# dek226/CSE375-FinalProj-Huffman-Decoding

Measured on AMD Instinct MI355X. Metric: decoded GB/s, higher is better.
Workload: dtype u8

## Files before the change

cse375-finalproj-huffman-decoding_amd/csrc/gh_decode.hip:

```cpp
#include <hip/hip_runtime.h>
#include <hip/hip_ext.h>

#include <algorithm>
#include <cmath>
#include <cstdio>
#include <cstring>
#include <map>
#include <memory>
#include <mutex>
#include <string>
#include <thread>
#include <type_traits>
#include <vector>

#include "gh_device.hpp"
#include "gh_gather_range.hpp"
#include "gh_hip.hpp"
#include "gh_internal.hpp"
#include "gh_lut.hpp"

namespace gh {

constexpr uint32_t EPOCH_MAX = (1u << 24) - 1;

#include "gh_tile.hip"
#include "gh_wsplit.hip"
#include "gh_index.hip"
#include "gh_gather.hip"
#include "gh_gather_plan.hip"
#include "gh_mtile.hip"

}

using namespace gh;

static uint32_t tile_u_for(uint32_t minlen) { return minlen >= 4 ? (uint32_t)TILE_U : (uint32_t)TILE_U3; }
#ifndef GH_TILE_OW7
#define GH_TILE_OW7 1
#endif
struct Kern {
  const void* fn;
  const char* name;
};
template <class... A>
static std::string kern_name(const char* fmt, A... a) {
  char b[96];
  snprintf(b, sizeof(b), fmt, a...);
  return b;
}
template <int TB, int U, int G, int OW, int MINL>
static Kern tile_kern() {
  static const std::string n = kern_name("tile<%d,%d,%d,%d,%d>", TB, U, G, OW, MINL);
  return {(const void*)gh_tile_kernel<TB, U, G, OW, MINL>, n.c_str()};
}
template <int TB, int GL, int NS, bool FB, int NP = 1>
static Kern mtile_kern() {
  static const std::string n = kern_name("mtile<%d,%d,%d,fb=%d,np=%d>", TB, GL, NS, (int)FB, NP);
  return {(const void*)gh_mtile_kernel<TB, GL, NS, FB, NP>, n.c_str()};
}
template <int U, int TB, int GL, bool FB>
static Kern ws_count_kern() {
  static const std::string n = kern_name("ws_count<%d,%d,%d,fb=%d>", U, TB, GL, (int)FB);
  return {(const void*)gh_ws_count_kernel<U, TB, GL, FB>, n.c_str()};
}
template <int U, int TB, int GL, int NS, bool FB>
static Kern ws_write_kern() {
  static const std::string n = kern_name("ws_write<%d,%d,%d,%d,fb=%d>", U, TB, GL, NS, (int)FB);
  return {(const void*)gh_ws_write_kernel<U, TB, GL, NS, FB>, n.c_str()};
}

static Kern tile_kernel_for(uint32_t minlen, uint32_t g) {
  if (minlen >= 5 && GH_TILE_OW7)
    return g >= 4 ? tile_kern<TILE_TB, TILE_U, 4, 7, 5>()
         : g == 3 ? tile_kern<TILE_TB, TILE_U, 3, 7, 5>()
                  : tile_kern<TILE_TB, TILE_U, 2, 7, 5>();
  if (minlen >= 4)
    return g >= 4 ? tile_kern<TILE_TB, TILE_U, 4, 8, 4>()
         : g == 3 ? tile_kern<TILE_TB, TILE_U, 3, 8, 4>()
                  : tile_kern<TILE_TB, TILE_U, 2, 8, 4>();
  return g >= 4 ? tile_kern<TILE_TB, TILE_U3, 4, 11, 3>()
       : g == 3 ? tile_kern<TILE_TB, TILE_U3, 3, 11, 3>()
                : tile_kern<TILE_TB, TILE_U3, 2, 11, 3>();
}

template <int GL, bool FB>
static Kern mtile_ns(int ns) {
  return ns <= 4 ? mtile_kern<MT_TB, GL, 4, FB>()
       : ns <= 6 ? mtile_kern<MT_TB, GL, 6, FB>()
       : ns <= 8 ? mtile_kern<MT_TB, GL, 8, FB>()
                 : mtile_kern<MT_TB, GL, 5, FB, 2>();
}
static Kern mtile_kernel_for(int gl, int ns, bool fb = false) {
  if (fb) return mtile_ns<2, true>(ns);
  return gl >= 4 ? mtile_ns<4, false>(ns) : gl == 3 ? mtile_ns<3, false>(ns) : mtile_ns<2, false>(ns);
}

struct WsKernels {
  Kern count;
  Kern write;
};
template <int GL, bool FB = false>
static Kern ws_write_ns(int ns) {
  return ns <= 2 ? ws_write_kern<WS_U, WS_TB, GL, 2, FB>()
         : ns <= 3 ? ws_write_kern<WS_U, WS_TB, GL, 3, FB>()
         : ns <= 4 ? ws_write_kern<WS_U, WS_TB, GL, 4, FB>()
         : ns <= 6 ? ws_write_kern<WS_U, WS_TB, GL, 6, FB>()
                   : ws_write_kern<WS_U, WS_TB, GL, 8, FB>();
}
template <class F>
static auto kernel_by_width(uint32_t bits, bool fb, F kern) {
  using std::integral_constant;
  if (fb) return kern(integral_constant<int, 2>{}, std::true_type{});
  const int gl = lookups_per_shift(bits);
  return gl >= 4 ? kern(integral_constant<int, 4>{}, std::false_type{})
       : gl == 3 ? kern(integral_constant<int, 3>{}, std::false_type{})
                 : kern(integral_constant<int, 2>{}, std::false_type{});
}
static WsKernels ws_kernels(uint32_t Kc, uint32_t K, int ns, bool fb) {
  return {kernel_by_width(Kc, fb, [](auto gl, auto f) { return ws_count_kern<WS_UC, WS_TBC, decltype(gl)::value, decltype(f)::value>(); }),
          kernel_by_width(K, fb, [ns](auto gl, auto f) { return ws_write_ns<decltype(gl)::value, decltype(f)::value>(ns); })};
}

static std::string all_kernel_shapes() {
  std::vector<std::string> v;
  auto add = [&](const char* n) {
    if (std::find(v.begin(), v.end(), n) == v.end()) v.push_back(n);
  };
  for (uint32_t ml = 3; ml <= 12; ++ml)
    for (uint32_t g = 2; g <= 4; ++g) add(tile_kernel_for(ml, g).name);
  for (int fb = 0; fb <= 1; ++fb)
    for (int gl = 2; gl <= 4; ++gl)
      for (int ns = 4; ns <= 10; ++ns) add(mtile_kernel_for(gl, ns, fb != 0).name);
  for (int pass = 0; pass < 2; ++pass)
    for (int fb = 0; fb <= 1; ++fb)
      for (uint32_t kc = 2; kc <= 14; ++kc)
        for (uint32_t k = 2; k <= 12; ++k)
          for (int ns = 2; ns <= 8; ++ns) {
            const WsKernels w = ws_kernels(kc, k, ns, fb != 0);
            add(pass ? w.write.name : w.count.name);
          }
  std::string s;
  for (const std::string& n : v) s += n + "\n";
  return s;
}

static_assert(TILE_U <= 4 && TILE_U3 <= 4, "payload padding (16 words) covers at most 4 segments per lane");


struct Shard {
  uint64_t nseg = 0, seg_begin = 0, seg_end = 0, n_total = 0, g_total = 0;
  uint32_t gap_nib0 = 0, first_start = 0;
  uint32_t last_end = 0;
  DevBuf payload;
  DevBuf gaps;
  DevBuf out;
  uint64_t out_cap = 0;
};

enum class Mode { NONE, TILE, MTILE, WSPLIT };

struct TilePlan {
  uint32_t ntiles = 0;
  uint32_t kbits = 0;
  uint32_t kbits_c = 0;
  uint32_t lut_lgr = 0;
  uint32_t clut_lgr = 0;
  uint32_t lut_bytes = 0;
  uint32_t stage_bytes = 0;
  uint32_t idle_block = 0xFFFFFFFFu;
  uint32_t epoch = 0;
  uint64_t gran_words = 0;
  DevBuf lut;
  DevBuf gran;
  DevBuf stamps;
};

struct WsPlan {
  Kern count{};
  uint32_t grid_c = 0;
  size_t lds_count = 0;
  uint32_t k = 0, kc = 0;
  uint32_t lgc = 0;
  uint32_t lut_bytes = 0;
  uint32_t stage_bytes = 0;
  uint32_t nblocks = 0, nranges = 0;
  DevBuf lut_c;
  DevBuf lut_w;
  DevBuf fb;
  DevBuf seg_cnt, junk, rng_tot, rng_off;
};

struct Plan {
  Mode mode = Mode::NONE;
  Kern kern{};
  uint32_t grid = 0, block = 0;
  size_t lds = 0;
  std::string shape;
  TilePlan tile;
  WsPlan ws;
  bool tiled() const { return mode == Mode::TILE || mode == Mode::MTILE; }
};

struct GatherTables {
  bool ready = false;
  uint32_t kc = 0, ks = 0;
  uint32_t last_end = 0;
  uint32_t wgs = 0;
  size_t lds = 0;
  const void* kern = nullptr;
  DevBuf lut_c;
  DevBuf lut_s;
  DevBuf fb;
};
struct Gather {
  GatherTables tab;
  DevBuf d_pieces, d_out;
  std::vector<gh_gather_piece> pieces;
  EventPair ev;
};
struct DevGather {
  bool has_index = false;
  uint32_t log2_stride = 0;
  uint64_t nblocks = 0;
  DevBuf offsets, rank;
  DevBuf loc, slot, dst0, pieces;
  Event ev_a, ev_b, ev_c;
  bool enqueued = false;
  hipStream_t last_stream = nullptr;
};

struct Timing {
  std::vector<EventPair> pending, pool;
  double acc_ms = 0;
  uint32_t nlaunch = 0;
};

struct gh_ctx {
  int device = 0;
  int num_cu = 0;
  Stream stream;
  Event done;
  bool done_rec = false;
  hipEvent_t done_ev = nullptr;
  bool loaded = false;
  Canon canon;
  DevBuf misc;
  Shard shard;
  Plan plan;
  Gather gather;
  DevGather dgather;
  Timing timing;
  ~gh_ctx();
  unsigned int* misc_at(int i) const { return misc.get<unsigned int>() + i; }
};

static void free_shard(gh_ctx* c) {
  (void)hipSetDevice(c->device);
  c->shard = Shard{};
  c->plan = Plan{};
  c->gather.tab = GatherTables{};
  c->dgather.has_index = false;
  c->dgather.offsets.reset();
  c->dgather.rank.reset();
  c->dgather.enqueued = false;
  c->loaded = false;
}

static int allow_lds(const void* fn, size_t lds) {
  if (lds > 64 * 1024) GH_HIP(hipFuncSetAttribute(fn, hipFuncAttributeMaxDynamicSharedMemorySize, (int)lds));
  return GH_OK;
}


static uint32_t tile_grid_cap(uint32_t grid) {
  if (const char* e = getenv("GH_TILE_GRID"))
    if (grid > 2) return (uint32_t)std::clamp<long>(atol(e), 2, (long)grid);
  return grid;
}

static int tile_grid_and_granules(Plan& p, uint64_t resident) {
  p.grid = (uint32_t)std::min<uint64_t>({(uint64_t)p.tile.ntiles + 1, resident, (uint64_t)LEAD_A * p.block});
  p.grid = tile_grid_cap(p.grid);
  if (p.grid < 2) return GH_OK;
  p.tile.gran_words = 2ull * p.tile.ntiles + 2;
  return p.tile.gran.alloc(8ull * p.tile.gran_words, true);
}

static int tile_setup(gh_ctx* c, uint32_t K, double avg_seg_bytes) {
  const Canon& cn = c->canon;
  Plan p;
  TilePlan& t = p.tile;
  const uint32_t maxsyms = (128 + cn.minlen - 1) / cn.minlen;
  t.kbits = K;
  const uint32_t tile_u = tile_u_for(cn.minlen);
  t.ntiles = (uint32_t)ceil_div(c->shard.nseg, (uint64_t)tile_u * TILE_TB);
  double scapf = 1.12;
  if (const char* e = getenv("GH_TILE_SCAPF")) scapf = std::clamp(atof(e), 0.5, 4.0);
  uint64_t per_seg = std::min<uint64_t>(
      maxsyms, cn.minlen >= 4 ? (uint64_t)TILE_SCAP : (uint64_t)std::ceil(std::max(avg_seg_bytes, 1.0) * scapf + 1));
  if (const char* e = getenv("GH_TILE_SCAP")) per_seg = std::min<uint64_t>(maxsyms, (uint64_t)std::max(1, atoi(e)));
  const uint64_t margin = 4ull * (cn.minlen >= 4 ? 8 : 11) + 4;
  const uint64_t seg_wave = 64ull * tile_u;
  per_seg = std::min<uint64_t>(per_seg, ((uint64_t)TILE_NS * 64 * 16 - 2 * STAGE_PAD - margin) / seg_wave);
  t.stage_bytes = (uint32_t)((STAGE_PAD + seg_wave * per_seg + margin + 15) & ~15ull);
  const std::vector<uint32_t> lt = grouped_lut(cn, K);
  p.kern = tile_kernel_for(cn.minlen, std::min<uint32_t>(4, 32 / cn.maxlen));
  p.block = TILE_TB;
  if (int rc = allow_lds(p.kern.fn, 160 * 1024)) return rc;
  const char* envr = getenv("GH_LGR");
  const int lg = envr ? std::clamp(atoi(envr), 0, 14 - (int)K) : std::min(5, 14 - (int)K);
  int best = 0, best_lg = 0;
  for (int l2 = lg; l2 >= 0; --l2) {
    int pc = 0;
    GH_HIP(hipOccupancyMaxActiveBlocksPerMultiprocessor(&pc, p.kern.fn, TILE_TB, tile_lds_bytes(4ull << (K + l2), t.stage_bytes)));
    if (pc > best) {
      best = pc;
      best_lg = l2;
    }
    if (envr) break;
  }
  best = std::min(best, 2);
  if (best < 1) return GH_OK;
  t.lut_lgr = (uint32_t)best_lg;
  t.lut_bytes = (uint32_t)(4ull << (K + best_lg));
  p.lds = tile_lds_bytes(t.lut_bytes, t.stage_bytes);
  if (int rc = tile_grid_and_granules(p, (uint64_t)best * c->num_cu)) return rc;
  if (p.grid < 2) return GH_OK;
  if (const char* e = getenv("GH_TILE_IDLE"))
    if (atoi(e) && p.grid == (uint32_t)best * c->num_cu && best == 2) t.idle_block = p.grid / 2;
  if (int rc = t.lut.upload(lt.data(), 4ull << K)) return rc;
  if (GH_TILE_STAMPS)
    if (int rc = t.stamps.alloc(32ull * p.grid * 2 * 128 + 8ull * (3ull * t.ntiles + 64 + 4 * 1024 + 4ull * p.grid), true))
      return rc;
  p.shape = p.kern.name;
  p.mode = Mode::TILE;
  c->plan = std::move(p);
  return GH_OK;
}

static uint32_t ws_write_bits(const Canon& cn);
static int mtile_setup(gh_ctx* c, double avg_seg_bytes) {
  const Canon& cn = c->canon;
  Plan p;
  TilePlan& t = p.tile;
  const bool one = cn.minlen == 1;
  const uint32_t K = one ? std::min<uint32_t>(ws_write_bits(cn), 11) : ws_write_bits(cn);
  const bool fb = K < cn.maxlen;
  if (fb && (K != (one ? 11u : 12u) || cn.maxlen > 16)) return GH_OK;
  const uint32_t maxsyms = (128 + cn.minlen - 1) / cn.minlen;
  double scapf = 1.12;
  if (const char* e = getenv("GH_TILE_SCAPF")) scapf = std::clamp(atof(e), 0.5, 4.0);
  uint64_t per_seg = std::min<uint64_t>(maxsyms, (uint64_t)std::ceil(std::max(avg_seg_bytes, 1.0) * scapf + 1));
  if (const char* e = getenv("GH_TILE_SCAP")) per_seg = std::min<uint64_t>(maxsyms, (uint64_t)std::max(1, atoi(e)));
  uint32_t Kc = K;
  if (GH_MT_CLUT && !one) {
    const int gl = lookups_per_shift(K);
    Kc = std::min<uint32_t>(13, 31 / gl);
    if (const char* e = getenv("GH_MT_KC")) Kc = (uint32_t)std::clamp(atoi(e), (int)K, (int)std::min(14, 31 / gl));
    Kc = std::max(Kc, K);
  }
  uint32_t clgr = 0;
  if (const char* e = getenv("GH_MT_CLGR")) clgr = (uint32_t)std::clamp(atoi(e), 0, 3);
  if (!GH_MT_CLUT || one) clgr = 0;
  clgr = std::min<uint32_t>(clgr, Kc + clgr > 14 ? 14 - Kc : clgr);
  const uint64_t lut_b = (GH_MT_CLUT ? (8ull << K) + (4ull << (Kc + clgr)) : 8ull << K)
                         + (fb ? (uint64_t)FB_BYTES : 0);
  const uint64_t lds_free = 160ull * 1024 - lut_b - mtile_lds_bytes(0, 0);
  const uint64_t region_max = std::min<uint64_t>(lds_free / (MT_TB / 64), (one ? 10 : 8) * 1024 + STAGE_PAD) & ~15ull;
  per_seg = std::min<uint64_t>(per_seg, (region_max - STAGE_PAD - 16) / (64ull * MT_U));
  {
    const uint64_t ps6 = (6144 - 16) / (64ull * MT_U);
    if (per_seg > ps6 && (double)ps6 >= std::max(avg_seg_bytes, 1.0) * 1.05 + 1) per_seg = ps6;
  }
  const uint64_t cap = std::max<uint64_t>(64ull * MT_U * per_seg, 64ull * maxsyms);
  if (STAGE_PAD + cap + 16 > region_max) return GH_OK;
  const int ns = cap + 16 <= 4096 ? 4 : cap + 16 <= 6144 ? 6 : cap + 16 <= 8192 ? 8 : 10;
  t.stage_bytes = (uint32_t)((STAGE_PAD + cap + 16 + 15) & ~15ull);
  p.kern = mtile_kernel_for(lookups_per_shift(K), ns, fb);
  p.block = MT_TB;
  t.lut_bytes = (uint32_t)lut_b;
  p.lds = mtile_lds_bytes(t.lut_bytes, t.stage_bytes);
  if (int rc = allow_lds(p.kern.fn, 160 * 1024)) return rc;
  int pc = 0;
  GH_HIP(hipOccupancyMaxActiveBlocksPerMultiprocessor(&pc, p.kern.fn, MT_TB, p.lds));
  pc = std::min(pc, 2);
  if (pc < 1) return GH_OK;
  t.kbits = K;
  t.kbits_c = Kc;
  t.clut_lgr = clgr;
  t.ntiles = (uint32_t)ceil_div(c->shard.nseg, (uint64_t)MT_U * MT_TB);
  if (int rc = tile_grid_and_granules(p, (uint64_t)pc * c->num_cu)) return rc;
  if (p.grid < 2) return GH_OK;
  std::vector<uint64_t> img(lut_b / 8, 0);
  const std::vector<uint64_t> lt = multi_lut(cn, K);
  const uint64_t wb = 8ull << K, cb = GH_MT_CLUT ? 4ull << (Kc + clgr) : 0;
  std::memcpy((uint8_t*)img.data() + (cb > wb ? cb : 0), lt.data(), wb);
  if (GH_MT_CLUT) {
    const std::vector<uint32_t> lc = start_count_lut(cn, Kc, clgr);
    std::memcpy((uint8_t*)img.data() + (cb > wb ? 0 : wb), lc.data(), cb);
  }
  if (fb) {
    uint32_t fbt[FB_WORDS];
    fallback_tables(cn, fbt);
    std::memcpy((uint8_t*)img.data() + lut_b - FB_BYTES, fbt, sizeof(fbt));
  }
  if (int rc = t.lut.upload(img.data(), lut_b)) return rc;
  p.shape = p.kern.name;
  p.mode = Mode::MTILE;
  c->plan = std::move(p);
  return GH_OK;
}

static uint32_t ws_count_bits(const Canon& cn) {
  const uint32_t lo = std::min<uint32_t>(std::max<uint32_t>(cn.maxlen, 2), 13);
  if (const char* e = getenv("GH_WS_KC")) return (uint32_t)std::clamp(atoi(e), (int)lo, 14);
  uint32_t best = lo;
  double best_eff = -1;
  for (uint32_t kc = lo; kc <= 13; ++kc) {
    const int gl = lookups_per_shift(kc);
    const double eff = gl * count_lut(cn, kc, nullptr) / (6.0 * gl + 8.0);
    if (eff > best_eff * 1.01) {
      best_eff = eff;
      best = kc;
    }
  }
  return best;
}
static uint32_t ws_write_bits(const Canon& cn) {
  if (const char* ek = getenv("GH_WS_K"))
    return (uint32_t)std::clamp(atoi(ek), 2, 12);
  const uint32_t lo = std::min<uint32_t>(std::max<uint32_t>(cn.maxlen, 10), 12);
  uint32_t best = lo;
  double best_eff = -1;
  for (uint32_t K = lo; K <= 12; ++K) {
    double sum = 0;
    for (uint32_t i = 0; i < (1u << K); ++i) sum += window_codewords(cn, i, K, 4, nullptr, nullptr, nullptr);
    const int gl = lookups_per_shift(K);
    const double eff = gl * (sum / (double)(1u << K)) / (13.0 * gl + 12.0);
    if (best_eff < 0 || eff > best_eff * 1.05) {
      best_eff = eff;
      best = K;
    }
  }
  return best;
}
#ifndef GH_WS_CLUT_MAX
#define GH_WS_CLUT_MAX 0
#endif
constexpr uint64_t WS_CLUT_MAX = GH_WS_CLUT_MAX;
static int ws_ns_for(double avg_seg_bytes) {
  const double chunks = avg_seg_bytes * 64 * WS_U / 16.0 * 1.15 + 2;
  const int ns = (int)std::ceil(chunks / 64);
  return ns <= 2 ? 2 : ns <= 3 ? 3 : ns <= 4 ? 4 : ns <= 6 ? 6 : 8;
}

static int upload_count_tables(const Canon& cn, uint32_t kc, DevBuf& lut_c, DevBuf& fb) {
  std::vector<uint32_t> lc;
  count_lut(cn, kc, &lc);
  uint32_t fbt[FB_WORDS];
  fallback_tables(cn, fbt);
  if (int rc = lut_c.upload(lc.data(), 4ull << kc)) return rc;
  return fb.upload(fbt, sizeof(fbt));
}

static int ws_setup(gh_ctx* c, double avg_seg_bytes) {
  const Canon& cn = c->canon;
  const uint64_t nseg = c->shard.nseg;
  Plan p;
  WsPlan& w = p.ws;
  const uint32_t K = ws_write_bits(cn), kc = ws_count_bits(cn);
  const bool fb = kraft16(cn) != 65536 || cn.maxlen > std::min(K, kc);
  w.k = K;
  w.kc = kc;
  if (int rc = w.lut_w.upload(write_lut(cn, K).data(), 8ull << K)) return rc;
  if (int rc = upload_count_tables(cn, kc, w.lut_c, w.fb)) return rc;
  w.lut_bytes = 8u << K;
  const size_t lb = w.lut_bytes + (fb ? (size_t)FB_BYTES : 0);
  constexpr int NW = WS_TB / 64;
  const uint32_t maxsyms = std::min<uint32_t>(143 / std::max<uint32_t>(cn.minlen, 1) + 1, 255);
  const size_t chain_worst = 64ull * maxsyms + 64;
  const size_t full_worst = 64ull * WS_U * maxsyms + 64;
  const size_t typical = (size_t)(1.3 * avg_seg_bytes * 64 * WS_U) + 64;
  const size_t want = std::max(chain_worst, std::min(full_worst, typical));
  size_t stage = 0;
  for (int wg = 8; wg >= 1 && stage == 0; --wg) {
    const long avail = ((long)(163840 / wg) - (long)lb) / NW;
    if (avail >= (long)want) stage = std::min<size_t>((size_t)avail, full_worst + 15) & ~15ull;
  }
  if (stage == 0) {
    const long avail = ((long)163840 - (long)lb) / NW;
    if (avail < (long)chain_worst) return fail(GH_E_HIP, "wave-split staging does not fit");
    stage = (size_t)avail & ~15ull;
  }
  if (const char* es = getenv("GH_WS_STAGE"))
    stage = std::max<size_t>((size_t)atoll(es), (chain_worst + 15) & ~15ull) & ~15ull;
  w.stage_bytes = (uint32_t)stage;
  p.lds = lb + NW * stage;
  if (!fb) {
    uint32_t lgc = 0;
    while (lgc < 5 && (4ull << (kc + lgc + 1)) <= (uint64_t)WS_CLUT_MAX && 30u - kc - (lgc + 1) >= 16u) ++lgc;
    if (const char* e = getenv("GH_WS_LGC")) lgc = (uint32_t)std::clamp(atoi(e), 0, std::max(0, 14 - (int)kc));
    w.lgc = lgc;
  }
  w.lds_count = std::max<size_t>(4ull << (kc + w.lgc), 64) + (fb ? FB_BYTES : 0);
  int ns = ws_ns_for(avg_seg_bytes);
  if (const char* en = getenv("GH_WS_NS")) ns = std::clamp(atoi(en), 2, 8);
  const WsKernels k = ws_kernels(kc, K, ns, fb);
  w.count = k.count;
  p.kern = k.write;
  p.block = WS_TB;
  if (int rc = allow_lds(w.count.fn, w.lds_count)) return rc;
  if (int rc = allow_lds(p.kern.fn, p.lds)) return rc;
  int pc_c = 0, pc_w = 0;
  GH_HIP(hipOccupancyMaxActiveBlocksPerMultiprocessor(&pc_c, w.count.fn, WS_TBC, w.lds_count));
  GH_HIP(hipOccupancyMaxActiveBlocksPerMultiprocessor(&pc_w, p.kern.fn, WS_TB, p.lds));
  if (pc_c < 1 || pc_w < 1) return fail(GH_E_HIP, "wave-split kernels do not fit on a CU");
  w.nblocks = (uint32_t)ceil_div(nseg, (uint64_t)WS_SB);
  const uint64_t wg_blocks = ceil_div(w.nblocks, (uint64_t)NW);
  p.grid = (uint32_t)std::min<uint64_t>((uint64_t)pc_w * c->num_cu, wg_blocks);
  w.grid_c = (uint32_t)std::min<uint64_t>((uint64_t)pc_c * c->num_cu, ceil_div(w.nblocks, (uint64_t)(WS_TBC / 64)));
  if (const char* eg = getenv("GH_WS_GRID")) {
    p.grid = (uint32_t)std::clamp<long>(atol(eg), 1, (long)p.grid);
    w.grid_c = (uint32_t)std::clamp<long>(atol(eg), 1, (long)w.grid_c);
  }
  w.nranges = p.grid * (uint32_t)NW;
  if (int rc = w.seg_cnt.alloc(nseg + WS_CNT_PAD + 16)) return rc;
  if (int rc = w.junk.alloc(16ull * 64 * w.nranges)) return rc;
  if (int rc = w.rng_tot.alloc(8ull * w.nranges + 16)) return rc;
  if (int rc = w.rng_off.alloc(8ull * w.nranges + 16)) return rc;
  p.shape = std::string(w.count.name) + "+" + p.kern.name;
  p.mode = Mode::WSPLIT;
  c->plan = std::move(p);
  return GH_OK;
}

static uint32_t last_segment_end(const Canon& cn, const uint32_t* w5, uint32_t start) {
  uint32_t pos = start;
  while (pos < 128) {
    const uint32_t wi = pos >> 5, sh = pos & 31;
    const uint32_t hi = w5[wi], lo = wi + 1 < 5 ? w5[wi + 1] : 0u;
    const uint32_t w32 = sh ? (hi << sh) | (lo >> (32 - sh)) : hi;
    uint32_t fi = 0;
    const uint32_t l = canon_decode16(cn, w32 >> 16, &fi);
    if (l == 0) break;
    pos += l;
  }
  return std::max<uint32_t>(pos, 128);
}

static uint32_t gap_nibble(const void* words, uint64_t nib) {
  uint32_t wv;
  std::memcpy(&wv, (const uint8_t*)words + 4 * (nib >> 3), 4);
  return (wv >> (4 * (nib & 7))) & 15u;
}

extern "C" int gh_device_count(void) {
  int n = 0;
  if (hipGetDeviceCount(&n) != hipSuccess) return 0;
  return n;
}

extern "C" int gh_ctx_create(int device, gh_ctx** out) {
  if (!out) return fail(GH_E_ARG, "null ctx pointer");
  *out = nullptr;
  int n = 0;
  if (hipGetDeviceCount(&n) != hipSuccess || n == 0)
    return fail(GH_E_NODEV, "no HIP device visible (the decoder has no CPU fallback)");
  if (device < 0 || device >= n) return fail(GH_E_ARG, "device ordinal out of range");
  hipDeviceProp_t prop;
  GH_HIP(hipGetDeviceProperties(&prop, device));
  if (std::string(prop.gcnArchName).find("gfx950") == std::string::npos)
    return fail(GH_E_NODEV, std::string("device is ") + prop.gcnArchName + ", need gfx950");
  std::unique_ptr<gh_ctx> c(new gh_ctx());
  c->device = device;
  c->num_cu = prop.multiProcessorCount;
  GH_HIP(hipSetDevice(device));
  if (int rc = c->stream.create()) return rc;
  if (int rc = c->done.create(hipEventDisableTiming)) return rc;
  if (int rc = c->misc.alloc(128, true)) return rc;
  *out = c.release();
  return GH_OK;
}

static int copy_name(const std::string& s, char* buf, size_t cap) {
  if (!buf) return fail(GH_E_ARG, "null argument");
  if (s.size() + 1 > cap) return fail(GH_E_SMALL, "name buffer too small");
  std::memcpy(buf, s.c_str(), s.size() + 1);
  return GH_OK;
}

extern "C" int gh_ctx_kernel_shape(gh_ctx* c, char* buf, size_t cap) {
  if (!c) return fail(GH_E_ARG, "null ctx");
  if (!c->loaded) return fail(GH_E_STATE, "gh_ctx_kernel_shape before gh_ctx_load");
  return copy_name(c->plan.shape, buf, cap);
}

extern "C" int gh_kernel_shapes(char* buf, size_t cap) { return copy_name(all_kernel_shapes(), buf, cap); }

extern "C" int gh_ctx_device(gh_ctx* c, int* device) {
  if (!c || !device) return fail(GH_E_ARG, "null argument");
  *device = c->device;
  return GH_OK;
}

struct DevChain {
  std::mutex mu;
  hipEvent_t last = nullptr;
  const gh_ctx* owner = nullptr;
  bool has = false;
  hipStream_t last_stream = nullptr;
};
static DevChain& dev_chain(int device) {
  static std::mutex mu;
  static std::map<int, DevChain*> m;
  std::lock_guard<std::mutex> g(mu);
  DevChain*& d = m[device];
  if (!d) d = new DevChain();
  return *d;
}

gh_ctx::~gh_ctx() {
  (void)hipSetDevice(device);
  if (stream) (void)hipStreamSynchronize(stream);
  if (done_rec) (void)hipEventSynchronize(done_ev);
  if (dgather.enqueued) (void)hipEventSynchronize(dgather.ev_c);
  DevChain& dc = dev_chain(device);
  std::lock_guard<std::mutex> g(dc.mu);
  if (dc.owner == this) {
    dc.has = false;
    dc.owner = nullptr;
    dc.last = nullptr;
  }
}

extern "C" int gh_ctx_destroy(gh_ctx* c) {
  delete c;
  return GH_OK;
}

static int plan_shard(gh_ctx* c, const gh_stream* s, uint64_t b, uint64_t e, uint64_t out_cap) {
  if (b > e || e > s->g) return fail(GH_E_ARG, "shard range outside [0, G]");
  if (e - b >= (1ull << 31))
    return fail(GH_E_ARG, "shard of 2^31 or more segments: split the stream into more shards");
  free_shard(c);
  int rc = build_canon(s->syms, s->nsyms, c->canon);
  if (rc) return rc;
  const Canon& cn = c->canon;
  Shard& sh = c->shard;
  sh.nseg = e - b;
  sh.seg_begin = b;
  sh.seg_end = e;
  sh.n_total = s->n;
  sh.g_total = s->g;
  if (sh.nseg > 0 && cn.nsyms == 0) return fail(GH_E_TABLE, "empty code");
  const uint64_t per_seg = cn.minlen ? (128 + cn.minlen - 1) / cn.minlen : 128;
  if (out_cap == 0) out_cap = std::min<uint64_t>(s->n, sh.nseg * per_seg);
  sh.out_cap = out_cap;
  GH_HIP(hipSetDevice(c->device));
  if ((rc = sh.out.alloc(std::max<uint64_t>(out_cap, 16) + 64))) return rc;
  GH_HIP(hipMemset(c->misc.get(), 0, 128));
  if (sh.nseg == 0) return GH_OK;
  const char* envm = getenv("GH_MODE");
  const bool force_tile = envm && !strcmp(envm, "tile"), force_ws = envm && !strcmp(envm, "wsplit");
  const bool force_mt = envm && !strcmp(envm, "mtile");
  if (envm && *envm && !force_tile && !force_ws && !force_mt) return fail(GH_E_ARG, "GH_MODE: tile, mtile or wsplit");
  const char* envk = getenv("GH_LUT_BITS");
  const uint32_t K = envk ? (uint32_t)std::clamp(atoi(envk), 1, 12) : cn.maxlen;
  const bool grouped = (grouped_code(cn) || short_code(cn)) && K >= cn.maxlen;
  if (force_tile && !grouped)
    return fail(GH_E_ARG, "GH_MODE=tile: the code is not for the tile kernel (complete, 3..12 bits)");
  const double avg = s->g ? (double)s->n / (double)s->g : 16.0;
  const Mode& mode = c->plan.mode;
  if (grouped && !force_ws && !force_mt) {
    if ((rc = tile_setup(c, K, avg))) return rc;
    if (force_tile && mode == Mode::NONE) return fail(GH_E_HIP, "GH_MODE=tile: the tile kernel does not fit a CU");
  }
  const bool multi = cn.maxlen <= 16 && kraft16(cn) == 65536;
  if (force_mt && !multi)
    return fail(GH_E_ARG, "GH_MODE=mtile: the code is not for the two-pass tile kernel (complete, 1..16 bits)");
  static const bool mt_on = [] {
    const char* e = getenv("GH_MTILE");
    return !(e && e[0] == '0');
  }();
  if (mode == Mode::NONE && multi && (force_mt || (mt_on && !force_ws && !force_tile))) {
    if ((rc = mtile_setup(c, avg))) return rc;
    if (force_mt && mode == Mode::NONE) return fail(GH_E_HIP, "GH_MODE=mtile: the two-pass tile kernel does not fit a CU");
  }
  if (mode == Mode::NONE) return ws_setup(c, avg);
  return GH_OK;
}

struct ShardSource {
  bool device;
  const void* payload;
  uint64_t skip, words;
  const void* gaps;
};

static int loaded_last_end(gh_ctx* c, uint32_t* out) {
  const Shard& sh = c->shard;
  uint32_t w5[5] = {};
  GH_HIP(hipMemcpy(w5, sh.payload.get<uint32_t>() + 4 * (sh.nseg - 1), sizeof(w5), hipMemcpyDeviceToHost));
  uint32_t st = sh.first_start;
  if (sh.nseg > 1) {
    const uint64_t nib = sh.gap_nib0 + sh.nseg - 2;
    uint32_t wv = 0;
    GH_HIP(hipMemcpy(&wv, sh.gaps.get<uint32_t>() + (nib >> 3), 4, hipMemcpyDeviceToHost));
    st = gap_nibble(&wv, nib & 7);
  }
  *out = last_segment_end(c->canon, w5, st);
  return GH_OK;
}

static int load_shard(gh_ctx* c, const gh_stream* s, uint64_t b, uint64_t e, uint64_t out_cap,
                      const ShardSource& src) {
  if (int rc = plan_shard(c, s, b, e, out_cap)) return rc;
  Shard& sh = c->shard;
  if (sh.nseg == 0) {
    c->loaded = true;
    return GH_OK;
  }
  const hipMemcpyKind kind = src.device ? hipMemcpyDeviceToDevice : hipMemcpyHostToDevice;
  const uint64_t have = std::min<uint64_t>(4 * sh.nseg + 1, src.skip < src.words ? src.words - src.skip : 0);
  const uint8_t* from = (const uint8_t*)src.payload + 4 * src.skip;
  const uint64_t alloc_words = 4 * sh.nseg + 16;
  if (int rc = sh.payload.alloc(4 * alloc_words)) return rc;
  GH_HIP(hipMemset(sh.payload.get<uint32_t>() + have, 0, 4 * (alloc_words - have)));
  if (have) {
    if (!src.device && use_staged(4 * have)) {
      if (int rc = h2d_staged(c->device, from, 4 * have, sh.payload.get())) return rc;
    } else {
      GH_HIP(hipMemcpy(sh.payload.get(), from, 4 * have, kind));
    }
  }
  const uint64_t gw0 = b >> 3;
  const uint64_t gw1 = (e >= 1) ? ((e - 1) >> 3) + 1 : gw0 + 1;
  const uint64_t gwords = std::max<uint64_t>(gw1, gw0 + 1) - gw0;
  const uint64_t total_gw = ceil_div(s->g, GH_GAPS_PER_WORD);
  const uint64_t gcopy = (gw0 < total_gw) ? std::min<uint64_t>(gwords, total_gw - gw0) : 0;
  if (int rc = sh.gaps.alloc(4 * (gwords + 4), true)) return rc;
  if (gcopy) GH_HIP(hipMemcpy(sh.gaps.get(), (const uint8_t*)src.gaps + 4 * gw0, 4 * gcopy, kind));
  sh.gap_nib0 = (uint32_t)(b - 8 * gw0);
  if (b > 0 && src.gaps) {
    if (src.device) {
      uint32_t wv = 0;
      GH_HIP(hipMemcpy(&wv, (const uint8_t*)src.gaps + 4 * ((b - 1) >> 3), 4, hipMemcpyDeviceToHost));
      sh.first_start = gap_nibble(&wv, (b - 1) & 7);
    } else {
      sh.first_start = gap_nibble(src.gaps, b - 1);
    }
  }
  if (c->plan.mode == Mode::WSPLIT && e == s->g)
    if (int rc = loaded_last_end(c, &sh.last_end)) return rc;
  c->loaded = true;
  return GH_OK;
}

extern "C" int gh_ctx_load(gh_ctx* c, const gh_stream* s, uint64_t b, uint64_t e,
                           uint64_t out_cap) {
  if (!c || !s) return fail(GH_E_ARG, "null argument");
  return load_shard(c, s, b, e, out_cap, {false, s->payload, 4 * b, s->w, s->gap_words});
}

extern "C" int gh_ctx_load_device(gh_ctx* c, const gh_stream* s, uint64_t b, uint64_t e,
                                  const uint32_t* d_payload, uint64_t d_words,
                                  const uint32_t* d_gap_words, uint64_t out_cap) {
  if (!d_payload || !d_gap_words) return fail(GH_E_ARG, "null device buffer");
  if (!c || !s) return fail(GH_E_ARG, "null argument");
  return load_shard(c, s, b, e, out_cap, {true, d_payload, 0, d_words, d_gap_words});
}

static WsParams shard_params(const gh_ctx* c) {
  const Shard& sh = c->shard;
  WsParams m{};
  m.payload = sh.payload.get<uint32_t>();
  m.gaps = sh.gaps.get<uint32_t>();
  m.nseg = (uint32_t)sh.nseg;
  m.gap_nib0 = sh.gap_nib0;
  m.first_start = sh.first_start;
  m.fb_lo = std::max<uint32_t>(c->canon.minlen, 1);
  m.fb_hi = std::max<uint32_t>(c->canon.maxlen, m.fb_lo);
  m.chk_pay = 4 * sh.nseg + 16;
  m.chk_gap = sh.nseg / 8 + 4;
  return m;
}

extern "C" int gh_ctx_decode(gh_ctx* c, void* hip_stream, int timed) {
  if (!c) return fail(GH_E_ARG, "null ctx");
  if (!c->loaded) return fail(GH_E_STATE, "gh_ctx_decode before gh_ctx_load");
  hipStream_t st = hip_stream ? (hipStream_t)hip_stream : (hipStream_t)c->stream;
  GH_HIP(hipSetDevice(c->device));
  const Shard& sh = c->shard;
  Plan& p = c->plan;
  if (sh.nseg == 0) {
    GH_HIP(hipMemsetAsync(c->misc_at(2), 0, 8, st));
    GH_HIP(hipEventRecord(c->done, st));
    c->done_ev = c->done;
    c->done_rec = true;
    return GH_OK;
  }
  const bool tiled = p.tiled();
  DevChain& dc = dev_chain(c->device);
  std::unique_lock<std::mutex> chain_lock(dc.mu, std::defer_lock);
  if (tiled) {
    if (++p.tile.epoch >= EPOCH_MAX) {
      GH_HIP(hipMemsetAsync(p.tile.gran.get(), 0, 8ull * p.tile.gran_words, st));
      p.tile.epoch = 1;
    }
    chain_lock.lock();
    const bool ordered = dc.owner == c && dc.last_stream == st && st == c->stream;
    if (dc.has && !ordered) GH_HIP(hipStreamWaitEvent(st, dc.last, 0));
  }
  EventPair ev;
  if (timed) {
    if (!c->timing.pool.empty()) {
      ev = std::move(c->timing.pool.back());
      c->timing.pool.pop_back();
    } else if (int rc = ev.create()) {
      return rc;
    }
    if (!tiled) GH_HIP(hipEventRecord(ev.a, st));
  }
  if (p.mode == Mode::WSPLIT) {
    const WsPlan& w = p.ws;
    WsParams m = shard_params(c);
    m.seg_cnt = w.seg_cnt.get<uint8_t>();
    m.rng_tot = w.rng_tot.get<unsigned long long>();
    m.rng_off = w.rng_off.get<unsigned long long>();
    m.out = sh.out.get<uint8_t>();
    m.junk = w.junk.get<uint4>();
    m.status = c->misc_at(1);
    m.total = (unsigned long long*)c->misc_at(2);
    m.out_cap = sh.out_cap;
    m.nsb = w.nblocks;
    m.nranges = w.nranges;
    m.chk_out = std::max<uint64_t>(sh.out_cap, 16) + 64;
    m.stage_bytes = w.stage_bytes;
    m.last_end = sh.last_end;
    m.fb = w.fb.get<uint32_t>();
    WsParams wc = m, ww = m;
    wc.lut = w.lut_c.get<uint2>();
    wc.kbits = w.kc;
    wc.lut_bytes = (uint32_t)(4u << w.kc);
    wc.lgc = w.lgc;
    ww.lut = w.lut_w.get<uint2>();
    ww.kbits = w.k;
    ww.lut_bytes = w.lut_bytes;
    void* ac[1] = {&wc};
    void* aw[1] = {&ww};
    GH_HIP(hipLaunchKernel(w.count.fn, dim3(w.grid_c), dim3(WS_TBC), ac, w.lds_count, st));
    GH_HIP(hipLaunchKernel((const void*)gh_ws_scan_kernel, dim3(1), dim3(WS_SCAN_TB), ac, 0, st));
    GH_HIP(hipLaunchKernel(p.kern.fn, dim3(p.grid), dim3(p.block), aw, p.lds, st));
  } else {
    const TilePlan& tp = p.tile;
    unsigned long long* gran = tp.gran.get<unsigned long long>();
    TileParams t{};
    t.payload = sh.payload.get<uint32_t>();
    t.gaps = sh.gaps.get<uint32_t>();
    t.lut = tp.lut.get<uint32_t>();
    t.out = sh.out.get<uint8_t>();
    t.granules = gran;
    t.prefix = gran + tp.ntiles;
    t.status = c->misc_at(1);
    t.total = (unsigned long long*)c->misc_at(2);
    t.stats = (unsigned long long*)c->misc_at(4);
    t.tickets = (unsigned int*)(gran + 2ull * tp.ntiles);
    t.out_cap = sh.out_cap;
    t.nseg = sh.nseg;
    t.gap_nib0 = sh.gap_nib0;
    t.first_start = sh.first_start;
    t.ntiles = tp.ntiles;
    t.kbits = tp.kbits;
    t.lgr = p.mode == Mode::MTILE ? tp.clut_lgr : tp.lut_lgr;
    t.epoch = tp.epoch;
    t.lut_bytes = tp.lut_bytes;
    t.stage_bytes = tp.stage_bytes;
    t.kbits_c = tp.kbits_c;
    t.fb_hi = c->canon.maxlen;
    t.stamps = tp.stamps.get<uint4>();
    t.tstamps = tp.stamps ? (unsigned long long*)(tp.stamps.get<uint8_t>() + 32ull * p.grid * 2 * 128) : nullptr;
    t.idle_block = tp.idle_block;
    void* ta[1] = {&t};
    if (timed)
      GH_HIP(hipExtLaunchKernel(p.kern.fn, dim3(p.grid), dim3(p.block), ta, p.lds, st, ev.a, ev.b, 0));
    else
      GH_HIP(hipLaunchKernel(p.kern.fn, dim3(p.grid), dim3(p.block), ta, p.lds, st));
  }
  GH_HIP(hipGetLastError());
  if (timed) {
    if (!tiled) GH_HIP(hipEventRecord(ev.b, st));
    c->done_ev = ev.b;
    c->timing.pending.push_back(std::move(ev));
  } else {
    GH_HIP(hipEventRecord(c->done, st));
    c->done_ev = c->done;
  }
  c->done_rec = true;
  if (tiled) {
    dc.last = c->done_ev;
    dc.owner = c;
    dc.has = true;
    dc.last_stream = st;
  }
  return GH_OK;
}

static int wait_decode(gh_ctx* c) {
  GH_HIP(hipStreamSynchronize(c->stream));
  if (c->done_rec) GH_HIP(hipEventSynchronize(c->done_ev));
  return GH_OK;
}

extern "C" int gh_ctx_report(gh_ctx* c, void* hip_stream, gh_report* rep) {
  if (!c) return fail(GH_E_ARG, "null ctx");
  hipStream_t st = hip_stream ? (hipStream_t)hip_stream : (hipStream_t)c->stream;
  GH_HIP(hipSetDevice(c->device));
  GH_HIP(hipStreamSynchronize(st));
  if (int rc = wait_decode(c)) return rc;
  Timing& tm = c->timing;
  for (EventPair& e : tm.pending) {
    float ms = 0;
    if (int rc = e.elapsed(&ms)) return rc;
    tm.acc_ms += ms;
    tm.nlaunch++;
    tm.pool.push_back(std::move(e));
  }
  tm.pending.clear();
  const Plan& p = c->plan;
  if (GH_TILE_STAMPS && p.tile.stamps) {
    if (const char* f = getenv("GH_STAMPS_OUT")) {
      std::vector<uint8_t> h(p.tile.stamps.capacity());
      GH_HIP(hipMemcpy(h.data(), p.tile.stamps.get(), h.size(), hipMemcpyDeviceToHost));
      if (FILE* fp = fopen(f, "wb")) {
        fwrite(h.data(), 1, h.size(), fp);
        fclose(fp);
      }
    }
  }
  unsigned int misc[6] = {};
  GH_HIP(hipMemcpy(misc, c->misc.get(), sizeof(misc), hipMemcpyDeviceToHost));
  if (rep) {
    std::memset(rep, 0, sizeof(*rep));
    uint64_t tot;
    std::memcpy(&tot, misc + 2, 8);
    rep->symbols = tot;
    rep->out_bytes = std::min<uint64_t>(tot, c->shard.out_cap);
    rep->status = misc[1];
    rep->lut_bits = p.tiled() ? p.tile.kbits : p.ws.k;
    rep->grid = p.grid;
    rep->tiles = p.tiled() ? p.tile.ntiles : p.ws.nblocks;
    rep->mode = p.mode == Mode::MTILE ? GH_MODE_MTILE : p.mode == Mode::TILE ? GH_MODE_TILE : GH_MODE_SPLIT;
    std::memcpy(&rep->slow_lookbacks, misc + 4, 8);
    rep->path = p.mode == Mode::MTILE ? GH_PATH_MULTI_TILE : p.mode == Mode::TILE ? GH_PATH_GROUPED : GH_PATH_MULTI_WAVE;
    rep->launches = tm.nlaunch;
    rep->kernel_ms = tm.nlaunch ? (float)(tm.acc_ms / tm.nlaunch) : 0.f;
  }
  return GH_OK;
}

extern "C" int gh_ctx_reset_timing(gh_ctx* c) {
  if (!c) return fail(GH_E_ARG, "null ctx");
  c->timing.acc_ms = 0;
  c->timing.nlaunch = 0;
  return GH_OK;
}

extern "C" int gh_ctx_download(gh_ctx* c, uint64_t off, uint8_t* dst, uint64_t nbytes) {
  if (!c || (nbytes && !dst)) return fail(GH_E_ARG, "null argument");
  if (off + nbytes > c->shard.out_cap) return fail(GH_E_ARG, "download beyond the output capacity");
  if (!nbytes) return GH_OK;
  GH_HIP(hipSetDevice(c->device));
  if (int rc = wait_decode(c)) return rc;
  const uint8_t* src = c->shard.out.get<uint8_t>() + off;
  if (use_staged(nbytes)) return d2h_staged(c->device, src, nbytes, dst);
  GH_HIP(hipMemcpy(dst, src, nbytes, hipMemcpyDeviceToHost));
  return GH_OK;
}

extern "C" int gh_ctx_output(gh_ctx* c, void** d_out, uint64_t* cap) {
  if (!c || !d_out) return fail(GH_E_ARG, "null argument");
  *d_out = c->shard.out.get();
  if (cap) *cap = c->shard.out_cap;
  return GH_OK;
}

extern "C" int gh_ctx_copy_output(gh_ctx* c, uint64_t off, void* dst, uint64_t nbytes,
                                  void* hip_stream) {
  if (!c || (nbytes && !dst)) return fail(GH_E_ARG, "null argument");
  if (off + nbytes > c->shard.out_cap) return fail(GH_E_ARG, "copy beyond the output capacity");
  if (!nbytes) return GH_OK;
  hipStream_t st = hip_stream ? (hipStream_t)hip_stream : (hipStream_t)c->stream;
  GH_HIP(hipSetDevice(c->device));
  if (c->done_rec) GH_HIP(hipStreamWaitEvent(st, c->done_ev, 0));
  GH_HIP(hipMemcpyAsync(dst, c->shard.out.get<uint8_t>() + off, nbytes, hipMemcpyDefault, st));
  return GH_OK;
}

extern "C" int gh_ctx_build_index(gh_ctx* c, uint32_t log2_stride, void* out, uint64_t out_len,
                                  uint64_t* symbols, float* kernel_ms) {
  if (!c || !out) return fail(GH_E_ARG, "null argument");
  if (!c->loaded) return fail(GH_E_STATE, "gh_ctx_build_index before gh_ctx_load");
  const Shard& sh = c->shard;
  const uint64_t bytes = gh_index_bytes(sh.g_total, log2_stride);
  if (bytes == 0) return fail(GH_E_ARG, "index stride outside 2^8 .. 2^20 segments");
  if (sh.seg_begin != 0 || sh.seg_end != sh.g_total)
    return fail(GH_E_ARG, "gh_ctx_build_index: the load must cover segments [0, G)");
  if (out_len < bytes) return fail(GH_E_SMALL, "index buffer smaller than gh_index_bytes");
  const uint64_t nblocks = (bytes - 40) / 8 - 1;
  std::vector<uint64_t> counts(nblocks, 0);
  float ms = 0;
  GH_HIP(hipSetDevice(c->device));
  if (int rc = wait_decode(c)) return rc;
  if (sh.nseg > 0) {
    const Canon& cn = c->canon;
    const uint32_t kc = ws_count_bits(cn);
    const bool fb = kraft16(cn) != 65536 || cn.maxlen > kc;
    DevBuf d_lut, d_fb, d_cnt, d_status;
    if (int rc = upload_count_tables(cn, kc, d_lut, d_fb)) return rc;
    if (int rc = d_cnt.alloc(8 * nblocks, true)) return rc;
    if (int rc = d_status.alloc(16, true)) return rc;
    IdxParams ip{};
    ip.w = shard_params(c);
    if (int rc = loaded_last_end(c, &ip.w.last_end)) return rc;
    ip.w.lut = d_lut.get<uint2>();
    ip.w.status = d_status.get<unsigned int>();
    ip.w.kbits = kc;
    ip.w.lut_bytes = (uint32_t)(4u << kc);
    ip.w.fb = d_fb.get<uint32_t>();
    ip.counts = d_cnt.get<unsigned long long>();
    ip.nblocks = (uint32_t)nblocks;
    ip.log2_stride = log2_stride;
    const void* kern = kernel_by_width(kc, fb, [](auto gl, auto f) {
      return (const void*)gh_index_count_kernel<IDX_U, IDX_TB, decltype(gl)::value, decltype(f)::value>;
    });
    const size_t lds = std::max<size_t>(4ull << kc, 64) + (fb ? FB_BYTES : 0);
    if (int rc = allow_lds(kern, lds)) return rc;
    int pc = 0;
    GH_HIP(hipOccupancyMaxActiveBlocksPerMultiprocessor(&pc, kern, IDX_TB, lds));
    if (pc < 1) return fail(GH_E_HIP, "the index kernel does not fit on a CU");
    uint32_t grid = (uint32_t)std::min<uint64_t>((uint64_t)pc * c->num_cu, ceil_div(nblocks, (uint64_t)(IDX_TB / 64)));
    if (const char* eg = getenv("GH_INDEX_GRID"))
      grid = (uint32_t)std::clamp<long>(atol(eg), 1, (long)grid);
    EventPair ev;
    if (int rc = ev.create()) return rc;
    void* args[1] = {&ip};
    {
      DevChain& dc = dev_chain(c->device);
      std::lock_guard<std::mutex> chain_lock(dc.mu);
      if (dc.has) GH_HIP(hipStreamWaitEvent(c->stream, dc.last, 0));
      GH_HIP(hipEventRecord(ev.a, c->stream));
      GH_HIP(hipLaunchKernel(kern, dim3(grid), dim3(IDX_TB), args, lds, c->stream));
      GH_HIP(hipGetLastError());
      GH_HIP(hipEventRecord(ev.b, c->stream));
      GH_HIP(hipStreamSynchronize(c->stream));
    }
    if (int rc = ev.elapsed(&ms)) return rc;
    unsigned int status = 0;
    GH_HIP(hipMemcpy(&status, d_status.get(), 4, hipMemcpyDeviceToHost));
    GH_HIP(hipMemcpy(counts.data(), d_cnt.get(), 8 * nblocks, hipMemcpyDeviceToHost));
    if (status & GH_ST_LAYOUT) return fail(GH_E_HIP, "index kernel: LDS layout assumption violated");
    if (status & GH_ST_BADCODE) return fail(GH_E_CORRUPT, "invalid code in stream");
  }
  uint8_t* o = (uint8_t*)out;
  auto put64 = [&](size_t at, uint64_t v) { std::memcpy(o + at, &v, 8); };
  uint64_t run = 0;
  for (uint64_t k = 0; k < nblocks; ++k) {
    if (run > sh.n_total) return fail(GH_E_CORRUPT, "stream holds more than N symbols before its last segments");
    put64(40 + 8 * k, run);
    run += counts[k];
  }
  if (run < sh.n_total) return fail(GH_E_CORRUPT, "stream holds fewer than N symbols");
  put64(40 + 8 * nblocks, sh.n_total);
  index_header(log2_stride, sh.n_total, sh.g_total, nblocks + 1, o);
  if (symbols) *symbols = run;
  if (kernel_ms) *kernel_ms = ms;
  return GH_OK;
}

static int gather_setup(gh_ctx* c) {
  const Canon& cn = c->canon;
  GatherTables t;
  t.kc = ws_count_bits(cn);
  t.ks = std::min<uint32_t>(std::max<uint32_t>(cn.maxlen, 2), 12);
  const bool fb = kraft16(cn) != 65536 || cn.maxlen > std::min(t.kc, t.ks);
  if (int rc = upload_count_tables(cn, t.kc, t.lut_c, t.fb)) return rc;
  if (int rc = t.lut_s.upload(single_lut(cn, t.ks).data(), 4ull << t.ks)) return rc;
  if (int rc = loaded_last_end(c, &t.last_end)) return rc;
  t.kern = kernel_by_width(t.kc, fb, [](auto gl, auto f) {
    return (const void*)gh_gather_kernel<GA_U, GA_TB, decltype(gl)::value, decltype(f)::value>;
  });
  t.lds = (4ull << t.kc) + (4ull << t.ks) + (fb ? FB_BYTES : 0);
  if (int rc = allow_lds(t.kern, t.lds)) return rc;
  int pc = 0;
  GH_HIP(hipOccupancyMaxActiveBlocksPerMultiprocessor(&pc, t.kern, GA_TB, t.lds));
  if (pc < 1) return fail(GH_E_HIP, "the gather kernel does not fit on a CU");
  t.wgs = (uint32_t)pc * (uint32_t)c->num_cu;
  if (int rc = c->gather.ev.create()) return rc;
  t.ready = true;
  c->gather.tab = std::move(t);
  return GH_OK;
}

extern "C" int gh_ctx_gather(gh_ctx* c, const gh_index* ix, const gh_range* ranges, uint32_t nranges,
                             void* dst, uint64_t dst_len, void* hip_stream, float* kernel_ms) {
  if (!c || !ix || !ix->offsets || (nranges && !ranges)) return fail(GH_E_ARG, "null argument");
  if (kernel_ms) *kernel_ms = 0;
  if (!c->loaded) return fail(GH_E_STATE, "gh_ctx_gather before gh_ctx_load");
  const Shard& sh = c->shard;
  Gather& ga = c->gather;
  if (sh.seg_begin != 0 || sh.seg_end != sh.g_total)
    return fail(GH_E_ARG, "gh_ctx_gather: the load must cover segments [0, G)");
  if (ix->n != sh.n_total || ix->g != sh.g_total) return fail(GH_E_ARG, "gh_ctx_gather: the index is another stream's (N, G)");
  const uint64_t ibytes = gh_index_bytes(ix->g, ix->log2_stride);
  if (ibytes == 0 || ix->nentries != (ibytes - 40) / 8) return fail(GH_E_ARG, "gh_ctx_gather: malformed index");
  uint64_t np = 0, total = 0;
  int rc = gh_gather_plan(ix, ranges, nranges, ga.pieces.data(), ga.pieces.size(), &np, &total);
  if (rc == GH_E_SMALL) {
    ga.pieces.resize(np);
    rc = gh_gather_plan(ix, ranges, nranges, ga.pieces.data(), ga.pieces.size(), &np, &total);
  }
  if (rc) return rc;
  if (total > dst_len) return fail(GH_E_SMALL, "gather destination smaller than the ranges' bytes");
  if (total == 0) return GH_OK;
  if (!dst) return fail(GH_E_ARG, "null argument");
  if (np >= (1ull << 31)) return fail(GH_E_ARG, "gh_ctx_gather: 2^31 or more pieces in one batch");
  hipStream_t st = hip_stream ? (hipStream_t)hip_stream : (hipStream_t)c->stream;
  GH_HIP(hipSetDevice(c->device));
  if (int rc2 = wait_decode(c)) return rc2;
  if (!ga.tab.ready)
    if (int rc2 = gather_setup(c)) return rc2;
  const GatherTables& t = ga.tab;
  if (int rc2 = ga.d_pieces.reserve(np * sizeof(gh_gather_piece))) return rc2;
  if (int rc2 = ga.d_out.reserve(total)) return rc2;
  unsigned int* d_status = c->misc_at(16);
  GatherParams gp{};
  gp.w = shard_params(c);
  gp.w.lut = t.lut_c.get<uint2>();
  gp.w.out = ga.d_out.get<uint8_t>();
  gp.w.status = d_status;
  gp.w.kbits = t.kc;
  gp.w.lut_bytes = (uint32_t)(4u << t.kc);
  gp.w.last_end = t.last_end;
  gp.w.fb = t.fb.get<uint32_t>();
  gp.pieces = ga.d_pieces.get<gh_gather_piece>();
  gp.sym_lut = t.lut_s.get<uint32_t>();
  gp.npieces = (uint32_t)np;
  gp.log2_stride = ix->log2_stride;
  gp.sym_bits = t.ks;
  uint32_t grid = (uint32_t)std::min<uint64_t>(t.wgs, ceil_div(np, (uint64_t)(GA_TB / 64)));
  if (const char* eg = getenv("GH_GATHER_GRID"))
    grid = (uint32_t)std::clamp<long>(atol(eg), 1, (long)grid);
  void* args[1] = {&gp};
  unsigned int status = 0;
  float ms = 0;
  {
    DevChain& dc = dev_chain(c->device);
    std::lock_guard<std::mutex> chain_lock(dc.mu);
    if (dc.has) GH_HIP(hipStreamWaitEvent(st, dc.last, 0));
    GH_HIP(hipMemsetAsync(d_status, 0, 4, st));
    GH_HIP(hipMemcpyAsync(ga.d_pieces.get(), ga.pieces.data(), np * sizeof(gh_gather_piece), hipMemcpyHostToDevice, st));
    GH_HIP(hipEventRecord(ga.ev.a, st));
    GH_HIP(hipLaunchKernel(t.kern, dim3(grid), dim3(GA_TB), args, t.lds, st));
    GH_HIP(hipGetLastError());
    GH_HIP(hipEventRecord(ga.ev.b, st));
    GH_HIP(hipMemcpyAsync(dst, ga.d_out.get(), total, hipMemcpyDefault, st));
    GH_HIP(hipStreamSynchronize(st));
  }
  if (int rc2 = ga.ev.elapsed(&ms)) return rc2;
  GH_HIP(hipMemcpy(&status, d_status, 4, hipMemcpyDeviceToHost));
  if (status & GH_ST_LAYOUT) return fail(GH_E_HIP, "gather kernel: LDS layout assumption violated");
  if (status & GH_ST_BADCODE) return fail(GH_E_CORRUPT, "gather: invalid code in stream, or the index is another stream's");
  if (kernel_ms) *kernel_ms = ms;
  return GH_OK;
}

extern "C" int gh_ctx_set_index(gh_ctx* c, const gh_index* ix) {
  if (!c || !ix || !ix->offsets) return fail(GH_E_ARG, "null argument");
  if (!c->loaded) return fail(GH_E_STATE, "gh_ctx_set_index before gh_ctx_load");
  const Shard& sh = c->shard;
  DevGather& dg = c->dgather;
  if (sh.seg_begin != 0 || sh.seg_end != sh.g_total)
    return fail(GH_E_ARG, "gh_ctx_set_index: the load must cover segments [0, G)");
  if (ix->n != sh.n_total || ix->g != sh.g_total) return fail(GH_E_ARG, "gh_ctx_set_index: the index is another stream's (N, G)");
  const uint64_t ibytes = gh_index_bytes(ix->g, ix->log2_stride);
  if (ibytes == 0 || ix->nentries != (ibytes - 40) / 8) return fail(GH_E_ARG, "gh_ctx_set_index: malformed index");
  std::vector<uint64_t> off(ix->nentries);
  std::memcpy(off.data(), ix->offsets, 8 * ix->nentries);
  const uint64_t nblocks = ix->nentries - 1;
  bool ok = off[0] == 0 && off[nblocks] == ix->n;
  for (uint64_t k = 0; k < nblocks && ok; ++k) ok = off[k + 1] >= off[k] && off[k + 1] - off[k] <= (143ull << ix->log2_stride);
  if (!ok) return fail(GH_E_ARG, "gh_ctx_set_index: the entries are not those of a parsed index");
  std::vector<uint32_t> rank(ix->nentries);
  gr_rank(off.data(), nblocks, rank.data());
  GH_HIP(hipSetDevice(c->device));
  if (dg.enqueued) GH_HIP(hipEventSynchronize(dg.ev_c));
  dg.has_index = false;
  if (int rc = dg.offsets.upload(off.data(), 8 * ix->nentries)) return rc;
  if (int rc = dg.rank.upload(rank.data(), 4 * ix->nentries)) return rc;
  dg.nblocks = nblocks;
  dg.log2_stride = ix->log2_stride;
  dg.has_index = true;
  return GH_OK;
}

extern "C" int gh_ctx_gather_device(gh_ctx* c, const gh_range* d_ranges, uint32_t nranges, void* d_dst,
                                    uint64_t dst_len, void* hip_stream) {
  if (!c) return fail(GH_E_ARG, "null ctx");
  if (!c->loaded) return fail(GH_E_STATE, "gh_ctx_gather_device before gh_ctx_load");
  DevGather& dg = c->dgather;
  if (!dg.has_index) return fail(GH_E_STATE, "gh_ctx_gather_device without a resident index (gh_ctx_set_index)");
  if (nranges == 0) return GH_OK;
  if (!d_ranges || !d_dst) return fail(GH_E_ARG, "null argument");
  if (nranges > GH_GATHER_MAX_RANGES) return fail(GH_E_ARG, "gh_ctx_gather_device: more than 2^24 ranges in one batch");
  const uint64_t cap = std::min<uint64_t>(gh_gather_piece_bound(nranges, dst_len, dg.log2_stride), (1ull << 31) - 1);
  hipStream_t st = hip_stream ? (hipStream_t)hip_stream : (hipStream_t)c->stream;
  GH_HIP(hipSetDevice(c->device));
  Gather& ga = c->gather;
  const bool has_segments = c->shard.nseg > 0;
  if (has_segments && !ga.tab.ready)
    if (int rc = gather_setup(c)) return rc;
  const GatherTables& t = ga.tab;
  if (int rc = dg.ev_a.create()) return rc;
  if (int rc = dg.ev_b.create()) return rc;
  if (int rc = dg.ev_c.create()) return rc;
  if (dg.loc.capacity() < nranges * sizeof(RangeLoc) || dg.pieces.capacity() < cap * sizeof(gh_gather_piece)) {
    if (dg.enqueued) GH_HIP(hipEventSynchronize(dg.ev_c));
    if (int rc = dg.loc.reserve(nranges * sizeof(RangeLoc))) return rc;
    if (int rc = dg.slot.reserve(nranges * 4ull)) return rc;
    if (int rc = dg.dst0.reserve(nranges * 8ull)) return rc;
    if (int rc = dg.pieces.reserve(cap * sizeof(gh_gather_piece))) return rc;
  }
  GplanParams pp{};
  pp.ranges = d_ranges;
  pp.offsets = dg.offsets.get<uint64_t>();
  pp.rank = dg.rank.get<uint32_t>();
  pp.loc = dg.loc.get<RangeLoc>();
  pp.slot = dg.slot.get<uint32_t>();
  pp.dst0 = dg.dst0.get<unsigned long long>();
  pp.pieces = dg.pieces.get<gh_gather_piece>();
  pp.status = c->misc_at(18);
  pp.npieces = c->misc_at(19);
  pp.totals = (unsigned long long*)c->misc_at(20);
  pp.nblocks = dg.nblocks;
  pp.n = c->shard.n_total;
  pp.cap = cap;
  pp.dst_len = dst_len;
  pp.nranges = nranges;
  GatherParams gp{};
  gp.w = shard_params(c);
  gp.w.lut = t.lut_c.get<uint2>();
  gp.w.out = (uint8_t*)d_dst;
  gp.w.status = pp.status;
  gp.w.kbits = t.kc;
  gp.w.lut_bytes = (uint32_t)(4u << t.kc);
  gp.w.last_end = t.last_end;
  gp.w.fb = t.fb.get<uint32_t>();
  gp.pieces = pp.pieces;
  gp.sym_lut = t.lut_s.get<uint32_t>();
  gp.d_npieces = pp.npieces;
  gp.log2_stride = dg.log2_stride;
  gp.sym_bits = t.ks;
  uint32_t grid = (uint32_t)std::min<uint64_t>(std::max<uint32_t>(t.wgs, 1), ceil_div(cap, (uint64_t)(GA_TB / 64)));
  if (const char* eg = getenv("GH_GATHER_GRID"))
    grid = (uint32_t)std::clamp<long>(atol(eg), 1, (long)grid);
  const uint32_t grid_r = (uint32_t)ceil_div((uint64_t)nranges, (uint64_t)GP_TB);
  const uint32_t grid_e = (uint32_t)std::min<uint64_t>(ceil_div(cap, (uint64_t)GP_TB), 1024);
  void* pa[1] = {&pp};
  void* args[1] = {&gp};
  DevChain& dc = dev_chain(c->device);
  std::lock_guard<std::mutex> chain_lock(dc.mu);
  const bool ordered = dc.owner == c && dc.last_stream == st && st == c->stream;
  if (dc.has && !ordered) GH_HIP(hipStreamWaitEvent(st, dc.last, 0));
  if (dg.enqueued && dg.last_stream != st) GH_HIP(hipStreamWaitEvent(st, dg.ev_c, 0));
  GH_HIP(hipEventRecord(dg.ev_a, st));
  GH_HIP(hipLaunchKernel((const void*)gh_gplan_locate_kernel, dim3(grid_r), dim3(GP_TB), pa, 0, st));
  GH_HIP(hipLaunchKernel((const void*)gh_gplan_scan_kernel, dim3(1), dim3(GP_SCAN_TB), pa, 0, st));
  GH_HIP(hipLaunchKernel((const void*)gh_gplan_emit_kernel, dim3(grid_e), dim3(GP_TB), pa, 0, st));
  GH_HIP(hipEventRecord(dg.ev_b, st));
  if (has_segments) GH_HIP(hipLaunchKernel(t.kern, dim3(grid), dim3(GA_TB), args, t.lds, st));
  GH_HIP(hipGetLastError());
  GH_HIP(hipEventRecord(dg.ev_c, st));
  dg.enqueued = true;
  dg.last_stream = st;
  dc.last = dg.ev_c;
  dc.owner = c;
  dc.has = true;
  dc.last_stream = st;
  return GH_OK;
}

static int dgather_result(gh_ctx* c, const char* who, unsigned int* status, uint64_t* np, uint64_t* bytes) {
  if (!c) return fail(GH_E_ARG, "null ctx");
  if (!c->dgather.enqueued) return fail(GH_E_STATE, std::string(who) + ": no device gather since the load");
  GH_HIP(hipSetDevice(c->device));
  GH_HIP(hipEventSynchronize(c->dgather.ev_c));
  unsigned int m[4] = {};
  GH_HIP(hipMemcpy(m, c->misc_at(18), sizeof(m), hipMemcpyDeviceToHost));
  *status = m[0];
  *np = m[1];
  std::memcpy(bytes, m + 2, 8);
  return GH_OK;
}

static int dgather_times(const gh_ctx* c, float* plan_ms, float* gather_ms) {
  GH_HIP(hipEventElapsedTime(plan_ms, c->dgather.ev_a, c->dgather.ev_b));
  GH_HIP(hipEventElapsedTime(gather_ms, c->dgather.ev_b, c->dgather.ev_c));
  return GH_OK;
}

extern "C" int gh_ctx_gather_times(gh_ctx* c, float* plan_ms, float* gather_ms) {
  unsigned int status;
  uint64_t np, bytes;
  if (int rc = dgather_result(c, "gh_ctx_gather_times", &status, &np, &bytes)) return rc;
  float a = 0, b = 0;
  if (int rc = dgather_times(c, &a, &b)) return rc;
  if (plan_ms) *plan_ms = a;
  if (gather_ms) *gather_ms = b;
  return GH_OK;
}

extern "C" int gh_ctx_gather_wait(gh_ctx* c, gh_gather_report* rep) {
  if (rep) std::memset(rep, 0, sizeof(*rep));
  unsigned int status;
  uint64_t np, bytes;
  if (int rc = dgather_result(c, "gh_ctx_gather_wait", &status, &np, &bytes)) return rc;
  float a = 0, b = 0;
  if (int rc = dgather_times(c, &a, &b)) return rc;
  if (rep) {
    rep->out_bytes = bytes;
    rep->npieces = np;
    rep->status = status;
    rep->kernel_ms = a + b;
  }
  if (status & GH_ST_RANGE) return fail(GH_E_ARG, "device gather: a byte range outside [0, N]");
  if (status & GH_ST_DSTSMALL) return fail(GH_E_SMALL, "device gather: destination smaller than the ranges' bytes");
  if (status & GH_ST_PIECES) return fail(GH_E_CORRUPT, "device gather: the plan exceeds the piece bound (the index is no real stream's)");
  if (status & GH_ST_LAYOUT) return fail(GH_E_HIP, "gather kernel: LDS layout assumption violated");
  if (status & GH_ST_BADCODE) return fail(GH_E_CORRUPT, "gather: invalid code in stream, or the index is another stream's");
  return GH_OK;
}

extern "C" int gh_ctx_gather_pieces(gh_ctx* c, gh_gather_piece* pieces, uint64_t cap, uint64_t* npieces) {
  if (!npieces || (cap && !pieces)) return fail(GH_E_ARG, "null argument");
  *npieces = 0;
  unsigned int status;
  uint64_t np, bytes;
  if (int rc = dgather_result(c, "gh_ctx_gather_pieces", &status, &np, &bytes)) return rc;
  *npieces = np;
  if (np > cap) return fail(GH_E_SMALL, "piece buffer smaller than the plan");
  if (np) GH_HIP(hipMemcpy(pieces, c->dgather.pieces.get(), np * sizeof(gh_gather_piece), hipMemcpyDeviceToHost));
  return GH_OK;
}

static float shards_kernel_ms(const std::vector<gh_ctx*>& ctx, const std::vector<gh_report>& reps) {
  std::map<int, float> per_dev;
  for (size_t k = 0; k < ctx.size(); ++k) per_dev[ctx[k]->device] += reps[k].kernel_ms;
  float worst = 0;
  for (auto& d : per_dev) worst = std::max(worst, d.second);
  return worst;
}

template <class F>
static int for_each_shard(int n, F f) {
  if (n == 1) return f(0);
  std::vector<int> rc(n, GH_OK);
  std::vector<std::string> msg(n);
  std::vector<std::thread> th;
  for (int k = 0; k < n; ++k)
    th.emplace_back([&, k] {
      rc[k] = f(k);
      if (rc[k]) msg[k] = gh_last_error();
    });
  for (auto& t : th) t.join();
  for (int k = 0; k < n; ++k)
    if (rc[k]) {
      set_error(msg[k]);
      return rc[k];
    }
  return GH_OK;
}

extern "C" int gh_decode(const gh_stream* s, uint8_t* out, uint64_t out_len, const gh_opts* o,
                         gh_report* rep) {
  if (!s || (s->n && !out)) return fail(GH_E_ARG, "null argument");
  if (out_len < s->n) return fail(GH_E_SMALL, "output buffer smaller than N");
  int rc = gh_stream_validate(s);
  if (rc) return rc;
  const int ng = (o && o->ngpus > 1) ? o->ngpus : 1;
  const int reps = (o && o->reps > 1) ? o->reps : 1;
  std::vector<uint64_t> bounds(ng + 1);
  gh_plan_shards(s->g, (uint32_t)ng, bounds.data());
  std::vector<gh_ctx*> ctx(ng, nullptr);
  auto cleanup = [&]() {
    for (auto* c : ctx) gh_ctx_destroy(c);
  };
  std::vector<gh_report> reps_k(ng);
  rc = for_each_shard(ng, [&](int k) {
    const int dev = (o && o->devices) ? o->devices[k] : (ng > 1 ? k : 0);
    int r = gh_ctx_create(dev, &ctx[k]);
    if (!r) r = gh_ctx_load(ctx[k], s, bounds[k], bounds[k + 1], ng > 1 ? 0 : s->n);
    for (int i = 0; i < reps && !r; ++i) r = gh_ctx_decode(ctx[k], nullptr, 1);
    if (!r) r = gh_ctx_report(ctx[k], nullptr, &reps_k[k]);
    return r;
  });
  if (rc) {
    cleanup();
    return rc;
  }
  std::vector<uint64_t> offs(ng + 1, 0), want(ng, 0);
  uint32_t status = 0;
  for (int k = 0; k < ng; ++k) {
    status |= reps_k[k].status;
    if (k + 1 < ng && reps_k[k].symbols > reps_k[k].out_bytes) {
      cleanup();
      return fail(GH_E_CORRUPT, "shard produced more symbols than its output capacity");
    }
    want[k] = (offs[k] < s->n) ? std::min<uint64_t>(reps_k[k].symbols, s->n - offs[k]) : 0;
    offs[k + 1] = offs[k] + reps_k[k].symbols;
  }
  const uint64_t offset = offs[ng];
  rc = for_each_shard(ng, [&](int k) { return want[k] ? gh_ctx_download(ctx[k], 0, out + offs[k], want[k]) : GH_OK; });
  const float dec_ms = shards_kernel_ms(ctx, reps_k);
  cleanup();
  if (rc) return rc;
  if (rep) {
    *rep = reps_k[0];
    rep->symbols = offset;
    rep->out_bytes = std::min<uint64_t>(offset, s->n);
    rep->status = status;
    rep->kernel_ms = dec_ms;
  }
  if (status & GH_ST_TIMEOUT) return fail(GH_E_HIP, "look-back timed out");
  if (offset < s->n) return fail(GH_E_CORRUPT, "stream decoded to fewer than N symbols");
  if (status & GH_ST_BADCODE) return fail(GH_E_CORRUPT, "invalid code in stream");
  return GH_OK;
}
```

cse375-finalproj-huffman-decoding_amd/csrc/gh_tile.hip:

```cpp

#ifndef GH_TILE_TB
#define GH_TILE_TB 1024
#endif
constexpr int TILE_TB = GH_TILE_TB;
#ifndef GH_TILE_U
#define GH_TILE_U 3
#endif
constexpr int TILE_U = GH_TILE_U;
constexpr int TILE_U3 = 2;
constexpr int TILE_NS = 4;
constexpr int TILE_SCAP = 20;
constexpr int TILE_MIDG = 2;
constexpr int STAGE_PAD = 16;
#ifndef GH_TILE_LAG
#define GH_TILE_LAG 2
#endif
constexpr int TILE_LAG = GH_TILE_LAG;
constexpr int TILE_SLOTS = 16;
#ifndef GH_TILE_STAMPS
#define GH_TILE_STAMPS 0
#endif
#if GH_TILE_STAMPS
#define TSTAMP(i) (ts[i] = __builtin_amdgcn_s_memtime())
#else
#define TSTAMP(i) ((void)0)
#endif
#ifndef GH_TILE_CSUB
#define GH_TILE_CSUB 0
#endif
#ifndef GH_TILE_CLDS
#define GH_TILE_CLDS 0
#endif
#ifndef GH_TILE_LMAJ
#define GH_TILE_LMAJ 1
#endif
#ifndef GH_TILE_POLLDIV
#define GH_TILE_POLLDIV 1
#endif
#ifndef GH_TILE_DYN
#define GH_TILE_DYN 0
#endif
constexpr int TILE_TAHEAD = 5;
#ifndef GH_TILE_LATEP
#define GH_TILE_LATEP 0
#endif
#ifndef GH_TILE_EPERM
#define GH_TILE_EPERM 0
#endif
#ifndef GH_TILE_HOLD
#define GH_TILE_HOLD 0
#endif
#ifndef GH_TILE_ALRD
#define GH_TILE_ALRD 1
#endif
#ifndef GH_TILE_W2
#define GH_TILE_W2 0
#endif
#ifndef GH_TILE_PF2
#define GH_TILE_PF2 0
#endif
#ifndef GH_TILE_ABLATE
#define GH_TILE_ABLATE 0
#endif
typedef unsigned int tile_v4u __attribute__((ext_vector_type(4)));
__device__ __forceinline__ void tile_st16(uint4* d, const uint4& v) {
  __builtin_nontemporal_store(tile_v4u{v.x, v.y, v.z, v.w}, (tile_v4u*)d);
}

struct TileParams {
  const uint32_t* payload;
  const uint32_t* gaps;
  const uint32_t* lut;
  uint8_t* out;
  unsigned long long* granules;
  unsigned long long* prefix;
  unsigned int* status;
  unsigned long long* total;
  unsigned long long* stats;
  unsigned long long out_cap;
  unsigned long long nseg;
  unsigned int gap_nib0, first_start, ntiles, kbits, lgr, epoch;
  unsigned int lut_bytes;
  unsigned int idle_block;
  unsigned int stage_bytes;
  unsigned int kbits_c;
  unsigned int fb_hi;
  unsigned int* tickets;
  uint4* stamps;
  unsigned long long* tstamps;
};

inline size_t tile_lds_bytes(size_t lut_bytes, size_t stage_bytes) {
  return lut_bytes + TILE_LAG * (TILE_TB / 64) * stage_bytes + TILE_SLOTS * (2 * (TILE_TB / 64) + 1) * 4 +
         TILE_SLOTS * 12 + 4 * (TILE_TB / 64) + 4 * TILE_SLOTS + 32;
}

__device__ __forceinline__ constexpr uint32_t perm_sel(int j) {
  return j == 0 ? 0x03020105u : j == 1 ? 0x03020500u : j == 2 ? 0x03050100u : 0x05020100u;
}

__device__ __forceinline__ void make_ewin(uint4 w, uint32_t w4, int start, uint32_t S, uint32_t (&e)[5]) {
  const uint32_t r = S - (uint32_t)start;
  e[0] = __builtin_amdgcn_alignbit(0u, w.x, r);
  e[1] = __builtin_amdgcn_alignbit(w.x, w.y, r);
  e[2] = __builtin_amdgcn_alignbit(w.y, w.z, r);
  e[3] = __builtin_amdgcn_alignbit(w.z, w.w, r);
  e[4] = __builtin_amdgcn_alignbit(w.w, w4, r);
}

constexpr uint32_t Q_SYMROOM = 0x7FFFu << 8;
constexpr uint32_t Q_LIVE = 128u << 23;
__device__ __forceinline__ uint32_t q_init(bool act, int start) {
  return ((act ? (uint32_t)(127 - start) : 511u) << 23) | Q_SYMROOM | 32u;
}

template <int N>
__device__ __forceinline__ void lds_wait_n(uint32_t& v) {
  static_assert(N >= 0 && N <= 3, "lgkmcnt 0..3");
  if constexpr (GH_TILE_CLDS) return;
  if constexpr (N == 0) asm volatile("s_waitcnt lgkmcnt(0)" : "+v"(v)::"memory");
  else if constexpr (N == 1) asm volatile("s_waitcnt lgkmcnt(1)" : "+v"(v)::"memory");
  else if constexpr (N == 2) asm volatile("s_waitcnt lgkmcnt(2)" : "+v"(v)::"memory");
  else asm volatile("s_waitcnt lgkmcnt(3)" : "+v"(v)::"memory");
}

template <int G, int U, int OW, int MINL, class Mid>
__device__ __forceinline__ int decode_tile_rolling(uint32_t (&e)[U][5], const int (&start)[U], const bool (&act)[U],
                                                   uint32_t (&ow)[U][OW], uint32_t (&cnt)[U], uint32_t amask,
                                                   uint32_t laneoff, Mid&& mid) {
  constexpr int S = 4 * OW;
  constexpr int NG = (S + G - 1) / G;
  constexpr int PLACE = GH_TILE_EPERM ? GH_TILE_EPERM : (G >= 4 ? 2 : 0);
  uint32_t q[U], ent[U];
#if GH_TILE_CLDS
  const __attribute__((address_space(3))) uint8_t* const lds0 = (const __attribute__((address_space(3))) uint8_t*)nullptr;
  auto lut_rd = [&](uint32_t a) -> uint32_t { return *(const __attribute__((address_space(3))) uint32_t*)(lds0 + a); };
#else
  auto lut_rd = [&](uint32_t a) -> uint32_t { return lds_u32_nowait(a); };
#endif
#pragma unroll
  for (int u = 0; u < U; ++u) {
    q[u] = q_init(act[u], start[u]);
    cnt[u] = 0;
#pragma unroll
    for (int k = 0; k < OW; ++k) asm volatile("" : "=v"(ow[u][k]));
  }
#pragma unroll
  for (int u = 0; u < U; ++u) ent[u] = lut_rd((e[u][0] & amask) | laneoff);
  int gdone = NG;
#pragma clang loop unroll(full)
  for (int gi = 0; gi < NG; ++gi) {
    const int CMIN = (gi + 1) * G * MINL;
    uint32_t qmin = 0xFFFFFFFFu;
#pragma clang loop unroll(full)
    for (int j = 0; j < G; ++j) {
      const int pos = gi * G + j;
      if (pos < S) {
        const bool gend = (j == G - 1) || (pos + 1 >= S);
        const bool last = gend && gi + 1 >= NG;
#pragma clang loop unroll(full)
        for (int u = 0; u < U; ++u) {
          if (last) {
            if constexpr (U == 3) {
              if (u == 0) lds_wait_n<2>(ent[u]);
              else if (u == 1) lds_wait_n<1>(ent[u]);
              else lds_wait_n<0>(ent[u]);
            } else if constexpr (U == 2) {
              if (u == 0) lds_wait_n<1>(ent[u]);
              else lds_wait_n<0>(ent[u]);
            } else {
              lds_wait_n<0>(ent[u]);
            }
          } else {
            lds_wait_n<U - 1>(ent[u]);
          }
#if GH_TILE_CSUB
          {
            uint32_t nq;
            const bool br = __builtin_sub_overflow(q[u], ent[u], &nq);
            q[u] = nq;
            cnt[u] = br ? (uint32_t)(pos + 1) : cnt[u];
          }
#else
          asm("v_sub_co_u32 %0, vcc, %0, %2\n\t"
              "v_cndmask_b32_e64 %1, %1, %3, vcc"
              : "+v"(q[u]), "+v"(cnt[u]) : "v"(ent[u]), "i"(pos + 1) : "vcc");
#endif
          ow[u][pos >> 2] = __builtin_amdgcn_perm(ent[u], ow[u][pos >> 2], perm_sel(pos & 3));
          if (PLACE == 1) asm volatile("" : "+v"(ow[u][pos >> 2]));
          if (!gend) {
            const uint32_t x = __builtin_amdgcn_alignbit(e[u][0], e[u][1], q[u]);
            ent[u] = lut_rd((x & amask) | laneoff);
          } else {
            e[u][0] = __builtin_amdgcn_alignbit(e[u][0], e[u][1], q[u]);
            if (CMIN + 32 < 157) e[u][1] = __builtin_amdgcn_alignbit(e[u][1], e[u][2], q[u]);
            if (CMIN + 64 < 157) e[u][2] = __builtin_amdgcn_alignbit(e[u][2], e[u][3], q[u]);
            if (CMIN + 96 < 157) e[u][3] = __builtin_amdgcn_alignbit(e[u][3], e[u][4], q[u]);
            if (CMIN + 128 < 157) e[u][4] = __builtin_amdgcn_alignbit(e[u][4], 0u, q[u]);
            q[u] = (q[u] & 0xFFFFFF00u) | 32u;
            qmin = min(qmin, q[u]);
            if (!last) ent[u] = lut_rd((e[u][0] & amask) | laneoff);
          }
        }
      }
    }
    if (PLACE == 2) {
#pragma unroll
      for (int u = 0; u < U; ++u) {
        const int w0 = (gi * G) >> 2, w1 = min(OW - 1, (gi * G + G - 1) >> 2);
#pragma unroll
        for (int wi = w0; wi <= w1; ++wi) asm volatile("" : "+v"(ow[u][wi]));
      }
    }
    if (gi == TILE_MIDG) mid();
    if (gi >= TILE_MIDG && gi + 1 < NG && !__any(qmin < Q_LIVE)) {
#pragma unroll
      for (int u = 0; u < U; ++u) lds_wait_n<0>(ent[u]);
      gdone = gi + 1;
      break;
    }
  }
  return gdone;
}

template <int OFF = 0>
__device__ __forceinline__ void lds_st32(uint32_t a, uint32_t v) {
  asm volatile("ds_write_b32 %0, %1 offset:%2" ::"v"(a), "v"(v), "i"(OFF) : "memory");
}
__device__ __forceinline__ uint32_t lds_ld_u32(uint32_t a) {
  uint32_t v;
  asm volatile("ds_read_b32 %0, %1\n\ts_waitcnt lgkmcnt(0)" : "=v"(v) : "v"(a) : "memory");
  return v;
}
__device__ __forceinline__ void lds_st_u32(uint32_t a, uint32_t v) {
  asm volatile("ds_write_b32 %0, %1\n\ts_waitcnt lgkmcnt(0)" ::"v"(a), "v"(v) : "memory");
}
__device__ __forceinline__ void lds_st32_m(uint32_t a, uint32_t v, int m) {
  switch (m) {
    case 1: lds_st32<4>(a, v); break;
    case 2: lds_st32<8>(a, v); break;
    case 3: lds_st32<12>(a, v); break;
    case 4: lds_st32<16>(a, v); break;
    case 5: lds_st32<20>(a, v); break;
    case 6: lds_st32<24>(a, v); break;
    case 7: lds_st32<28>(a, v); break;
    case 8: lds_st32<32>(a, v); break;
    case 9: lds_st32<36>(a, v); break;
    case 10: lds_st32<40>(a, v); break;
    case 11: lds_st32<44>(a, v); break;
    default: lds_st32<0>(a + 4u * (uint32_t)m, v); break;
  }
}
template <int U, int OW>
__device__ __forceinline__ void stage_wave(const uint32_t (&ow)[U][OW], const uint32_t (&n)[U], const uint32_t (&o)[U],
                                           int mmax) {
  uint32_t base[U], sh[U];
#pragma unroll
  for (int u = 0; u < U; ++u) {
    const uint32_t ap = ((o[u] - 1u) & 3u) + 1u;
    base[u] = o[u] - ap;
    sh[u] = 4u - ap;
  }
  auto dw = [&](int u, int m) { return __builtin_amdgcn_alignbyte(m < OW ? ow[u][m] : 0u, ow[u][m - 1], sh[u]); };
  if constexpr (GH_TILE_W2) {
#pragma unroll
    for (int m = OW; m >= 1; m -= 2) {
      if (m - 1 >= 1) {
        if (m <= mmax) {
#pragma unroll
          for (int u = 0; u < U; ++u)
            asm volatile("ds_write2_b32 %0, %1, %2 offset0:%3 offset1:%4" ::"v"(base[u]), "v"(dw(u, m)),
                         "v"(dw(u, m - 1)), "i"(m), "i"(m - 1) : "memory");
        } else if (m - 1 <= mmax) {
#pragma unroll
          for (int u = 0; u < U; ++u) lds_st32_m(base[u], dw(u, m - 1), m - 1);
        }
      } else if (m <= mmax) {
#pragma unroll
        for (int u = 0; u < U; ++u) lds_st32_m(base[u], dw(u, m), m);
      }
    }
  } else {
#pragma unroll
    for (int m = OW; m >= 1; --m) {
      if (m > mmax) continue;
#pragma unroll
      for (int u = 0; u < U; ++u) lds_st32_m(base[u], dw(u, m), m);
    }
  }
  uint32_t rd[U];
#pragma unroll
  for (int u = 0; u < U; ++u) rd[u] = lds_u32_nowait(base[u]);
  lds_wait(rd);
#pragma unroll
  for (int u = 0; u < U; ++u) {
    const uint32_t ap = o[u] - base[u];
    if (n[u] && ap < 4u) {
      const uint32_t ab = 8u * ap;
      lds_st32(base[u], (rd[u] & ((1u << ab) - 1u)) | (ow[u][0] << ab));
    }
  }
}

constexpr uint32_t OOB_OFF = 0x80000000u;
template <int NS, bool PIN = true>
__device__ __forceinline__ void copy_out_piece(uint8_t* out, uint32_t stg, unsigned long long goff, uint32_t n,
                                               int lane, tile_v4u (&v)[NS], uint32_t& b, uint32_t c0 = 0) {
  goff = rfl_u64(goff);
  n = (uint32_t)__builtin_amdgcn_readfirstlane((int)n);
  const uint32_t lb = (uint32_t)(goff & 15);
  const __amdgpu_buffer_rsrc_t rs = __builtin_amdgcn_make_buffer_rsrc(out + (goff - lb), 0, 0x7FFFFFF0, 0x00020000);
  const uint32_t src = (stg + 16u - ((GH_TILE_ABLATE & 128) ? 0u : lb)) & ((GH_TILE_ABLATE & 256) ? ~3u : ~0u);
  const uint32_t cf = lb ? 1u : 0u;
  const uint32_t ce = n ? (lb + n) >> 4 : 0u;
  uint32_t off[NS];
#pragma unroll
  for (int i = 0; i < NS; ++i) {
    const uint32_t c = c0 + cf + (uint32_t)lane + 64u * (uint32_t)i;
    off[i] = c < ce ? 16u * c : OOB_OFF;
  }
  const uint32_t nh = (lb && n) ? min(16u, lb + n) - lb : 0u;
  const uint32_t tl = (lb + n) & 15u;
  const uint32_t nt = (n && tl && (ce > 0 || !lb)) ? tl : 0u;
  const uint32_t t = (uint32_t)lane;
  uint32_t k = OOB_OFF;
  if (c0 == 0u && !(GH_TILE_ABLATE & 64)) {
    if (t < nh) k = lb + t;
    else if (t < nh + nt) k = 16u * ce + (t - nh);
  }
  if constexpr (GH_TILE_ALRD) {
    constexpr int CG = NS % 2 == 0 ? 2 : 1;
    const uint32_t sh = (16u - lb) & 15u, r = sh & 3u, m = lb ? sh >> 2 : 4u;
    if constexpr (GH_TILE_ALRD == 2) {
      tile_v4u P[NS + 1];
#pragma unroll
      for (int i = 0; i <= NS; ++i) {
        const uint32_t c = c0 + cf + (uint32_t)lane + 64u * (uint32_t)i;
        const uint32_t a = stg + 16u * (c < ce + 1u ? c : cf);
        asm volatile("ds_read_b128 %0, %1" : "=v"(P[i]) : "v"(a) : "memory");
      }
      if (PIN) asm volatile("ds_read_u8 %0, %1" : "+v"(b) : "v"(src + (k == OOB_OFF ? 0u : k)) : "memory");
      else asm volatile("ds_read_u8 %0, %1" : "=v"(b) : "v"(src + (k == OOB_OFF ? 0u : k)) : "memory");
      asm volatile("s_waitcnt lgkmcnt(0)" ::: "memory");
#pragma unroll
      for (int i = 0; i <= NS; ++i) asm volatile("" : "+v"(P[i]));
#pragma unroll
      for (int i = 0; i < NS; ++i) {
        tile_v4u Q;
#pragma unroll
        for (int d = 0; d < 4; ++d) {
          const int nx = __builtin_amdgcn_update_dpp(0, (int)P[i + 1][d], 0x134, 0xf, 0xf, false);
          Q[d] = (uint32_t)__builtin_amdgcn_update_dpp(nx, (int)P[i][d], 0x130, 0xf, 0xf, false);
        }
        auto W = [&](int q) -> uint32_t { return q < 4 ? P[i][q] : Q[q - 4]; };
        switch (m) {
          case 0:
            for (int d = 0; d < 4; ++d) v[i][d] = __builtin_amdgcn_alignbyte(W(d + 1), W(d), r);
            break;
          case 1:
            for (int d = 0; d < 4; ++d) v[i][d] = __builtin_amdgcn_alignbyte(W(d + 2), W(d + 1), r);
            break;
          case 2:
            for (int d = 0; d < 4; ++d) v[i][d] = __builtin_amdgcn_alignbyte(W(d + 3), W(d + 2), r);
            break;
          case 3:
            for (int d = 0; d < 4; ++d) v[i][d] = __builtin_amdgcn_alignbyte(W(d + 4), W(d + 3), r);
            break;
          default:
            v[i] = Q;
            break;
        }
        __builtin_amdgcn_raw_buffer_store_b128(v[i], rs, (int)off[i], 0, 2);
      }
      if (PIN) asm volatile("" : "+v"(b));
      __builtin_amdgcn_raw_buffer_store_b8((uint8_t)b, rs, (int)k, 0, 2);
      return;
    }
#pragma unroll
    for (int g0 = 0; g0 < NS; g0 += CG) {
      tile_v4u pq[CG][2];
#pragma unroll
      for (int j = 0; j < CG; ++j) {
        const int i = g0 + j;
        const uint32_t c = c0 + cf + (uint32_t)lane + 64u * (uint32_t)i;
        const uint32_t a = stg + 16u * (c < ce ? c : cf);
        asm volatile("ds_read_b128 %0, %1" : "=v"(pq[j][0]) : "v"(a) : "memory");
        asm volatile("ds_read_b128 %0, %1 offset:16" : "=v"(pq[j][1]) : "v"(a) : "memory");
      }
      if (g0 + CG >= NS) {
        if (PIN) asm volatile("ds_read_u8 %0, %1" : "+v"(b) : "v"(src + (k == OOB_OFF ? 0u : k)) : "memory");
        else asm volatile("ds_read_u8 %0, %1" : "=v"(b) : "v"(src + (k == OOB_OFF ? 0u : k)) : "memory");
      }
      asm volatile("s_waitcnt lgkmcnt(0)" ::: "memory");
#pragma unroll
      for (int j = 0; j < CG; ++j) asm volatile("" : "+v"(pq[j][0]), "+v"(pq[j][1]));
      auto shift = [&](auto mc) {
        constexpr int M = decltype(mc)::value;
#pragma unroll
        for (int j = 0; j < CG; ++j) {
          if constexpr (M == 4) {
            v[g0 + j] = pq[j][1];
          } else {
            auto W = [&](int q) -> uint32_t { return q < 4 ? pq[j][0][q] : pq[j][1][q - 4]; };
#pragma unroll
            for (int d = 0; d < 4; ++d) v[g0 + j][d] = __builtin_amdgcn_alignbyte(W(M + d + 1), W(M + d), r);
          }
        }
      };
      switch (m) {
        case 0: shift(std::integral_constant<int, 0>{}); break;
        case 1: shift(std::integral_constant<int, 1>{}); break;
        case 2: shift(std::integral_constant<int, 2>{}); break;
        case 3: shift(std::integral_constant<int, 3>{}); break;
        default: shift(std::integral_constant<int, 4>{}); break;
      }
#pragma unroll
      for (int j = 0; j < CG; ++j) __builtin_amdgcn_raw_buffer_store_b128(v[g0 + j], rs, (int)off[g0 + j], 0, 2);
    }
    if (PIN) asm volatile("" : "+v"(b));
    __builtin_amdgcn_raw_buffer_store_b8((uint8_t)b, rs, (int)k, 0, 2);
    return;
  }
#pragma unroll
  for (int i = 0; i < NS; ++i) {
    const uint32_t c = c0 + cf + (uint32_t)lane + 64u * (uint32_t)i;
    if (PIN) asm volatile("ds_read_b128 %0, %1" : "+v"(v[i]) : "v"(src + 16u * (c < ce ? c : cf)) : "memory");
    else asm volatile("ds_read_b128 %0, %1" : "=v"(v[i]) : "v"(src + 16u * (c < ce ? c : cf)) : "memory");
  }
  if (PIN) asm volatile("ds_read_u8 %0, %1" : "+v"(b) : "v"(src + (k == OOB_OFF ? 0u : k)) : "memory");
  else asm volatile("ds_read_u8 %0, %1" : "=v"(b) : "v"(src + (k == OOB_OFF ? 0u : k)) : "memory");
  asm volatile("s_waitcnt lgkmcnt(0)" : "+v"(b)::"memory");
#pragma unroll
  for (int i = 0; i < NS; ++i) asm volatile("" : "+v"(v[i]));
#pragma unroll
  for (int i = 0; i < NS; ++i) __builtin_amdgcn_raw_buffer_store_b128(v[i], rs, (int)off[i], 0, 2);
  __builtin_amdgcn_raw_buffer_store_b8((uint8_t)b, rs, (int)k, 0, 2);
}

template <int OW>
__device__ __forceinline__ void store_direct(uint8_t* out, unsigned long long cap, unsigned long long o,
                                             const uint32_t (&ow)[OW], uint32_t n) {
#pragma unroll
  for (int i = 0; i < 4 * OW; ++i)
    if ((uint32_t)i < n && o + (uint32_t)i < cap) out[o + (uint32_t)i] = (uint8_t)(ow[i >> 2] >> (8 * (i & 3)));
}

__device__ __forceinline__ bool granule_ok(const TileParams& p, unsigned long long v, uint32_t flag) {
  return (uint32_t)(v >> 40) == p.epoch && (uint32_t)((v >> 38) & 3u) == flag;
}

__device__ __forceinline__ unsigned long long poll_granule(const TileParams& p, unsigned long long* g,
                                                           uint32_t flag) {
  unsigned long long t0 = 0;
  for (uint32_t spins = 1;; ++spins) {
    const unsigned long long v = __hip_atomic_load(g, __ATOMIC_RELAXED, __HIP_MEMORY_SCOPE_AGENT);
    if (granule_ok(p, v, flag)) return v;
    if ((spins & 63u) == 0u) {
      if (__hip_atomic_load(p.status, __ATOMIC_RELAXED, __HIP_MEMORY_SCOPE_AGENT) & GH_ST_TIMEOUT) return 0;
      const unsigned long long t = wall_clock64();
      if (t0 == 0) {
        t0 = t;
      } else if (t - t0 > 400000000ull) {
        atomicOr(p.status, (unsigned)GH_ST_TIMEOUT);
        return 0;
      }
    }
    __builtin_amdgcn_s_sleep(2);
  }
}

constexpr int LEAD_A = 4;
template <int TB>
__device__ __forceinline__ void tile_round_leader(const TileParams& p, uint32_t D, uint32_t* s_lead, int tid,
                                                  int lane, int wid) {
  const uint32_t A = (D + TB - 1) / TB;
  const uint32_t nr = (p.ntiles + D - 1) / D;
  unsigned long long R = 0;
  for (uint32_t r = 0; r < nr; ++r) {
    const uint32_t t0 = r * D, n = min(D, p.ntiles - t0);
    uint32_t v[LEAD_A], sum = 0;
#pragma unroll
    for (int i = 0; i < LEAD_A; ++i) {
      const uint32_t j = (uint32_t)tid * A + (uint32_t)i;
      v[i] = 0;
      if ((uint32_t)i < A && j < n) {
        unsigned long long g = __hip_atomic_load(&p.granules[t0 + j], __ATOMIC_RELAXED, __HIP_MEMORY_SCOPE_AGENT);
        if (!granule_ok(p, g, 1)) {
          atomicAdd(p.stats + 1, 1ull);
          g = poll_granule(p, &p.granules[t0 + j], 1);
        }
        v[i] = (uint32_t)(g & GRAN_VMASK);
      }
      sum += v[i];
    }
    const uint32_t incl = wave_incl_scan(sum);
    if (lane == 63) s_lead[wid] = incl;
    __syncthreads();
    unsigned long long before = 0, total = 0;
#pragma unroll
    for (int q = 0; q < TB / 64; ++q) {
      const uint32_t x = s_lead[q];
      before += (q < wid) ? x : 0u;
      total += x;
    }
    unsigned long long run = R + before + incl - sum;
#pragma unroll
    for (int i = 0; i < LEAD_A; ++i) {
      const uint32_t j = (uint32_t)tid * A + (uint32_t)i;
      if ((uint32_t)i < A && j < n)
        __hip_atomic_store(&p.prefix[t0 + j], granule(p.epoch, 2, run), __ATOMIC_RELAXED, __HIP_MEMORY_SCOPE_AGENT);
      run += v[i];
    }
    R += total;
#if GH_TILE_STAMPS
    if (tid == 0) p.tstamps[2 * p.ntiles + r] = __builtin_amdgcn_s_memrealtime();
#endif
    __syncthreads();
  }
}

template <int TB>
__device__ __forceinline__ void tile_frontier_leader(const TileParams& p, uint32_t* s_w, int tid, int lane, int wid) {
  constexpr int NW = TB / 64;
  uint32_t F = 0;
  unsigned long long R = 0, t0 = 0;
  uint32_t* const s_first = s_w;
  uint32_t* const s_sum = s_w + 2 * NW;
  for (uint32_t pass = 0; F < p.ntiles; ++pass) {
    const uint32_t t = F + (uint32_t)tid, pb = (pass & 1u) * NW;
    bool in = false;
    uint32_t v = 0;
    if (t < p.ntiles) {
      const unsigned long long g = __hip_atomic_load(&p.granules[t], __ATOMIC_RELAXED, __HIP_MEMORY_SCOPE_AGENT);
      in = granule_ok(p, g, 1);
      v = (uint32_t)(g & GRAN_VMASK);
    }
    const unsigned long long out = __ballot(!in);
    if (lane == 0) s_first[pb + wid] = out ? (uint32_t)__builtin_ctzll(out) : 64u;
    __syncthreads();
    uint32_t m = (uint32_t)TB;
#pragma unroll
    for (int q = NW - 1; q >= 0; --q) {
      const uint32_t f = s_first[pb + q];
      m = f < 64u ? 64u * (uint32_t)q + f : m;
    }
    const uint32_t vv = (uint32_t)tid < m ? v : 0u;
    const uint32_t incl = wave_incl_scan(vv);
    if (lane == 63) s_sum[pb + wid] = incl;
    __syncthreads();
    unsigned long long before = 0, total = 0;
#pragma unroll
    for (int q = 0; q < NW; ++q) {
      const uint32_t x = s_sum[pb + q];
      before += (q < wid) ? x : 0u;
      total += x;
    }
    if ((uint32_t)tid < m) {
      __hip_atomic_store(&p.prefix[t], granule(p.epoch, 2, R + before + incl - vv), __ATOMIC_RELAXED,
                         __HIP_MEMORY_SCOPE_AGENT);
#if GH_TILE_STAMPS
      p.tstamps[2 * p.ntiles + t] = __builtin_amdgcn_s_memrealtime();
#endif
    }
    R += total;
    F += m;
    if (m == 0u) {
      if (tid == 0) atomicAdd(p.stats + 1, 1ull);
      if ((pass & 63u) == 0u) {
        if (__hip_atomic_load(p.status, __ATOMIC_RELAXED, __HIP_MEMORY_SCOPE_AGENT) & GH_ST_TIMEOUT) return;
        const unsigned long long tw = wall_clock64();
        if (t0 == 0) {
          t0 = tw;
        } else if (tw - t0 > 400000000ull) {
          if (tid == 0) atomicOr(p.status, (unsigned)GH_ST_TIMEOUT);
          return;
        }
      }
      __builtin_amdgcn_s_sleep(2);
    } else {
      t0 = 0;
    }
  }
}

template <int TB, int U, int GRP, int OW, int MINL>
__global__ __launch_bounds__(TB) __attribute__((amdgpu_waves_per_eu(4, 4))) void gh_tile_kernel(const TileParams p) {
  static_assert(4 * OW >= (128 + MINL - 1) / MINL, "OW words hold every codeword a segment can start");
  static_assert(U <= TILE_U, "shapes of at most TILE_U segments per lane");
  constexpr int NW = TB / 64;
  extern __shared__ __attribute__((aligned(16))) uint8_t smem[];
  const uint32_t stage_lds = p.lut_bytes;
  uint32_t* s_tot = (uint32_t*)(smem + p.lut_bytes + TILE_LAG * NW * p.stage_bytes);
  uint32_t* s_off = s_tot + TILE_SLOTS * NW;
  uint32_t* s_cnt = s_off + TILE_SLOTS * NW;
  unsigned long long* s_pfx = (unsigned long long*)(s_cnt + TILE_SLOTS);
  uint32_t* s_ptile = (uint32_t*)(s_pfx + TILE_SLOTS);
  uint32_t* s_lead = s_ptile + TILE_SLOTS;
  uint32_t* s_ring = s_lead + NW;
  const uint32_t cnt_lds = (uint32_t)((uint8_t*)s_cnt - smem);
  const uint32_t ptile_lds = (uint32_t)((uint8_t*)s_ptile - smem);
  const uint32_t ring_lds = (uint32_t)((uint8_t*)s_ring - smem);

  const int tid = threadIdx.x, lane = tid & 63, wid = tid >> 6;
#if GH_TILE_STAMPS
  unsigned long long* const lring = p.tstamps + 3ull * p.ntiles + 64 + 4ull * (p.epoch & 1023u);
  if (blockIdx.x == 0 && tid == 0) {
    lring[0] = __builtin_amdgcn_s_memtime();
    lring[1] = __builtin_amdgcn_s_memrealtime();
  }
#endif
  const uint32_t D = gridDim.x - 1 - (p.idle_block < gridDim.x ? 1u : 0u);
  if (blockIdx.x == 0) {
    if constexpr (GH_TILE_DYN) {
      if (tid == 0) p.tickets[2u * ((p.epoch + 1u) & 1u)] = 0u;
      tile_frontier_leader<TB>(p, (uint32_t*)smem, tid, lane, wid);
    } else {
      tile_round_leader<TB>(p, D, s_lead, tid, lane, wid);
    }
#if GH_TILE_STAMPS
    if (tid == 0) {
      lring[2] = __builtin_amdgcn_s_memtime();
      lring[3] = __builtin_amdgcn_s_memrealtime();
    }
#endif
    return;
  }
  if (blockIdx.x == p.idle_block) return;
#if GH_TILE_STAMPS
  unsigned long long* const wring = p.tstamps + 3ull * p.ntiles + 64 + 4ull * 1024 + 4ull * blockIdx.x;
  if (tid == 0) {
    wring[0] = __builtin_amdgcn_s_memtime();
    wring[1] = __builtin_amdgcn_s_memrealtime();
  }
#endif
  {
    const uint32_t nd = p.lut_bytes >> 2;
    uint32_t* sl = (uint32_t*)smem;
    for (uint32_t i = tid; i < nd; i += TB) sl[i] = p.lut[i >> p.lgr];
    if (tid < TILE_SLOTS) {
      s_cnt[tid] = 0;
      s_ptile[tid] = 0xFFFFFFFFu;
    }
    if (GH_TILE_DYN && tid <= TILE_TAHEAD) {
      const uint32_t b0 = blockIdx.x - 1 - (blockIdx.x > p.idle_block ? 1u : 0u);
      const uint32_t tt = b0 + (uint32_t)tid * D;
      s_ring[tid] = tt < p.ntiles ? tt : 0xFFFFFFFFu;
    }
  }
  const uint32_t S = 30u - p.kbits - p.lgr;
  const uint32_t amask = (((1u << p.kbits) - 1u) << (2u + p.lgr)) & ((GH_TILE_ABLATE & 16) ? ~(1u << (2u + p.lgr)) : ~0u);
  const uint32_t laneoff = ((uint32_t)lane & ((1u << p.lgr) - 1u)) << 2;
  check_lds_base(smem, p.status);

  const uint32_t G = D, b = blockIdx.x - 1 - (blockIdx.x > p.idle_block ? 1u : 0u);
  const uint32_t nseg = (uint32_t)p.nseg;
  constexpr uint32_t NONE = 0xFFFFFFFFu;
  __syncthreads();
  const uint32_t last_tile_k = GH_TILE_DYN ? p.ntiles + 2u * TILE_SLOTS
                               : b < p.ntiles ? (p.ntiles - 1 - b) / G : NONE;
  uint32_t cur = b, nxt = b + G;
  const uint32_t dyn_base = (uint32_t)(TILE_TAHEAD + 1) * D;
  uint32_t tk = 0;
  bool tk_live = GH_TILE_DYN && dyn_base < p.ntiles;
  unsigned int* const tctr = GH_TILE_DYN ? p.tickets + 2u * (p.epoch & 1u) : nullptr;
  constexpr uint32_t CSTR = GH_TILE_LMAJ ? 1u : 64u;
  const uint32_t lseg = (uint32_t)(wid * 64 * U) + (uint32_t)lane * (GH_TILE_LMAJ ? (uint32_t)U : 1u);
  constexpr int NSET = GH_TILE_PF2 ? 2 : 1;
  static_assert(!(GH_TILE_PF2 && (GH_TILE_DYN || GH_TILE_HOLD)), "PF2: static schedule, no hold");
  uint4 wset[NSET][U];
  uint32_t w4set[NSET][U], gwset[NSET][U];
  auto load = [&](auto SS, uint32_t t) {
    constexpr int SI = decltype(SS)::value;
    uint4 (&w)[U] = wset[SI];
    uint32_t (&w4)[U] = w4set[SI];
    uint32_t (&gw)[U] = gwset[SI];
    const uint32_t seg0 = min(t, p.ntiles - 1) * (uint32_t)(U * TB) + lseg;
    if constexpr (GH_TILE_LMAJ) {
      const uint32_t sb = min(seg0, nseg - 1);
#pragma unroll
      for (int u = 0; u < U; ++u) w[u] = *(const uint4*)(p.payload + 4ull * (sb + (uint32_t)u));
      w4[U - 1] = p.payload[4ull * (sb + (uint32_t)U)];
#pragma unroll
      for (int u = 0; u < U; ++u) {
        const uint32_t sc = sb + (uint32_t)u;
        gw[u] = p.gaps[(p.gap_nib0 + (sc ? sc - 1u : 0u)) >> 3];
      }
    } else {
#pragma unroll
      for (int u = 0; u < U; ++u) {
        const uint32_t sc = min(seg0 + (uint32_t)(64 * u), nseg - 1);
        w[u] = *(const uint4*)(p.payload + 4ull * sc);
        w4[u] = p.payload[4ull * sc + 4];
        gw[u] = p.gaps[(p.gap_nib0 + (sc ? sc - 1u : 0u)) >> 3];
      }
    }
  };
  const __amdgpu_buffer_rsrc_t rs_out = __builtin_amdgcn_make_buffer_rsrc(p.out, 0, 0x7FFFFFF0, 0x00020000);
  auto ticket_op = [&]() {
    if constexpr (GH_TILE_DYN) {
      if (wid == 0 && tk_live) {
        if (lane == 0) tk = atomicAdd(tctr, 1u);
      } else {
        __builtin_amdgcn_raw_buffer_store_b8((uint8_t)0, rs_out, (int)(OOB_OFF + 64u), 0, 2);
      }
    }
  };
  auto junk_stores = [&]() {
    const __amdgpu_buffer_rsrc_t rs = rs_out;
#pragma unroll
    for (int i = 0; i < TILE_NS; ++i)
      __builtin_amdgcn_raw_buffer_store_b128(tile_v4u{0, 0, 0, 0}, rs, (int)(OOB_OFF + 16u * (uint32_t)i), 0, 2);
    __builtin_amdgcn_raw_buffer_store_b8((uint8_t)0, rs, (int)OOB_OFF, 0, 2);
  };
  load(std::integral_constant<int, 0>{}, cur);
  ticket_op();
  junk_stores();
  if constexpr (GH_TILE_PF2) {
    (void)__hip_atomic_load(&p.prefix[0], __ATOMIC_RELAXED, __HIP_MEMORY_SCOPE_AGENT);
    (void)__hip_atomic_load(&p.prefix[0], __ATOMIC_RELAXED, __HIP_MEMORY_SCOPE_AGENT);
    load(std::integral_constant<int, NSET - 1>{}, nxt);
    junk_stores();
  }
  if (cur >= p.ntiles) cur = NONE;
  uint32_t th[TILE_LAG];
#pragma unroll
  for (int i = 0; i < TILE_LAG; ++i) th[i] = NONE;
  uint32_t owp[U][OW], cntp[U], bposp[U], wtp = 0, prevt = NONE;
  int gdp = 1;
#pragma unroll
  for (int u = 0; u < U; ++u) {
    cntp[u] = 0;
    bposp[u] = 0;
#pragma unroll
    for (int k2 = 0; k2 < OW; ++k2) asm volatile("" : "=v"(owp[u][k2]));
  }
  uint32_t rank = 0;
  const uint32_t region0 = stage_lds + (uint32_t)wid * p.stage_bytes;
  const uint32_t piece_cap = p.stage_bytes - (uint32_t)(STAGE_PAD + 4 * OW + 4);
#if GH_TILE_STAMPS
  unsigned long long ts[9];
#endif
  auto body = [&](auto SS, uint32_t k) -> bool {
    constexpr int SI = decltype(SS)::value;
    uint4 (&w)[U] = wset[SI];
    uint32_t (&w4)[U] = w4set[SI];
    uint32_t (&gw)[U] = gwset[SI];
    TSTAMP(0);
    const bool have_cur = cur < p.ntiles;
    const uint32_t t2 = th[TILE_LAG - 1];
    const bool have2 = t2 < p.ntiles;
    bool pending = have_cur || (GH_TILE_HOLD && prevt < p.ntiles);
#pragma unroll
    for (int i = 0; i < TILE_LAG; ++i) pending |= th[i] < p.ntiles;
    if (!pending) return false;
    if (last_tile_k != NONE && k > last_tile_k + TILE_LAG + 2) {
      if (lane == 0) atomicOr(p.status, (unsigned)GH_ST_TIMEOUT);
      return false;
    }
    const uint32_t slot = k % TILE_SLOTS, slot2 = (k + TILE_SLOTS - TILE_LAG - GH_TILE_HOLD) % TILE_SLOTS;
    const uint32_t slotp = (k + TILE_SLOTS - 1) % TILE_SLOTS;
    const uint32_t buf = k % TILE_LAG;
    if (rank >= 3) __builtin_amdgcn_s_setprio(3);
    else if (rank == 2) __builtin_amdgcn_s_setprio(2);
    else if (rank == 1) __builtin_amdgcn_s_setprio(1);
    else __builtin_amdgcn_s_setprio(0);
    unsigned long long* const pf2 = &p.prefix[have2 ? t2 : 0u];
    unsigned long long gp0 = 0, gp = 0, gpl = 0;
    if (!(GH_TILE_ABLATE & 4)) gp0 = __hip_atomic_load(pf2, __ATOMIC_RELAXED, __HIP_MEMORY_SCOPE_AGENT);
    auto mid = [&]() {
      if (!(GH_TILE_ABLATE & 4)) gp = __hip_atomic_load(pf2, __ATOMIC_RELAXED, __HIP_MEMORY_SCOPE_AGENT);
    };
    const uint32_t seg0 = cur * (uint32_t)(U * TB) + lseg;
    uint32_t ow[U][OW], cnt[U];
    int gdone;
    {
      int start[U];
      bool act[U];
      uint32_t e[U][5];
#pragma unroll
      for (int u = 0; u < U; ++u) {
        const uint32_t seg = seg0 + (uint32_t)u * CSTR;
        act[u] = have_cur && seg < nseg;
        start[u] = seg == 0 ? (int)p.first_start : (int)gap_nib(gw[u], p.gap_nib0 + seg - 1u);
        make_ewin(w[u], (GH_TILE_LMAJ && u + 1 < U) ? w[u + 1 < U ? u + 1 : u].x : w4[u], start[u], S, e[u]);
      }
      TSTAMP(1);
      if (GH_TILE_ABLATE & 1) {
#pragma unroll
        for (int u = 0; u < U; ++u) {
          cnt[u] = act[u] ? 16u : 0u;
#pragma unroll
          for (int k2 = 0; k2 < OW; ++k2) ow[u][k2] = e[u][k2 % 5];
        }
        mid();
        gdone = (16 + GRP - 1) / GRP;
      } else {
        gdone = decode_tile_rolling<GRP, U, OW, MINL>(e, start, act, ow, cnt, amask, laneoff, mid);
      }
    }
    if constexpr (GH_TILE_DYN) {
      if (wid == 0) {
        uint32_t tpost = NONE;
        if (lane == 0 && tk_live) tpost = dyn_base + tk < p.ntiles ? dyn_base + tk : NONE;
        tpost = (uint32_t)__builtin_amdgcn_readfirstlane((int)tpost);
        tk_live = tk_live && tpost != NONE;
        if (lane == 0) lds_st_u32(ring_lds + 4u * ((k + 1u + TILE_TAHEAD) % TILE_SLOTS), tpost);
      }
      nxt = lds_ld_u32(ring_lds + 4u * ((k + 1u) % TILE_SLOTS));
      nxt = (uint32_t)__builtin_amdgcn_readfirstlane((int)nxt);
    }
    if (GH_TILE_LATEP && !(GH_TILE_ABLATE & 4)) gpl = __hip_atomic_load(pf2, __ATOMIC_RELAXED, __HIP_MEMORY_SCOPE_AGENT);
    load(SS, GH_TILE_PF2 ? nxt + G : nxt);
    ticket_op();
    TSTAMP(2);
    uint32_t bpos[U], wave_tot = 0;
    if constexpr (GH_TILE_LMAJ) {
      uint32_t sl = 0;
#pragma unroll
      for (int u = 0; u < U; ++u) sl += cnt[u];
      const uint32_t incl = wave_incl_scan(sl);
      uint32_t run = incl - sl;
#pragma unroll
      for (int u = 0; u < U; ++u) {
        bpos[u] = run;
        run += cnt[u];
      }
      wave_tot = (uint32_t)__builtin_amdgcn_readlane((int)incl, 63);
    } else {
#pragma unroll
      for (int u = 0; u < U; ++u) bpos[u] = wave_incl_scan(cnt[u]);
#pragma unroll
      for (int u = 0; u < U; ++u) {
        const uint32_t ct = (uint32_t)__builtin_amdgcn_readlane((int)bpos[u], 63);
        bpos[u] += wave_tot - cnt[u];
        wave_tot += ct;
      }
    }
    uint32_t tile_total = 0;
    if (have_cur) {
      uint32_t old = 0;
      if (lane == 0) {
        s_tot[slot * NW + wid] = wave_tot;
        asm volatile("ds_add_rtn_u32 %0, %1, %2\n\ts_waitcnt lgkmcnt(0)" : "=v"(old) : "v"(cnt_lds + 4u * slot), "v"(1u)
                     : "memory");
      }
      const uint32_t arr = (uint32_t)__builtin_amdgcn_readfirstlane((int)old);
      rank = (4u * arr) / NW;
      if (arr == NW - 1) {
        const uint32_t x = lane < NW ? s_tot[slot * NW + lane] : 0u;
        const uint32_t xi = wave_incl_scan(x);
        if (lane < NW) s_off[slot * NW + lane] = xi - x;
        tile_total = (uint32_t)__builtin_amdgcn_readlane((int)xi, NW - 1);
        if (lane == 0) {
          s_cnt[slot] = 0;
          asm volatile("s_waitcnt lgkmcnt(0)" ::: "memory");
          __hip_atomic_store(&p.granules[cur], granule(p.epoch, 1, tile_total), __ATOMIC_RELAXED,
                             __HIP_MEMORY_SCOPE_AGENT);
#if GH_TILE_STAMPS
          p.tstamps[cur] = __builtin_amdgcn_s_memrealtime();
#endif
        }
      }
    }
    TSTAMP(3);
    unsigned long long goff = 0;
    uint32_t n2 = 0;
    if (have2 && (GH_TILE_ABLATE & 4)) {
      goff = ((unsigned long long)t2 * (U * TB * 16) + (uint32_t)wid * (U * 64 * 16)) % (p.out_cap - (U * TB * 32));
      n2 = s_tot[slot2 * NW + wid];
    } else if (have2) {
      unsigned long long g = rfl_u64(gp0);
      bool polled = false, got = true;
      (void)polled;
      if (!granule_ok(p, g, 2)) g = rfl_u64(gp);
      if (GH_TILE_LATEP && !granule_ok(p, g, 2)) g = rfl_u64(gpl);
      {
        if (!granule_ok(p, g, 2)) {
          polled = true;
          if (wid == 0 && lane == 0) atomicAdd(p.stats, 1ull);
          unsigned long long t0w = 0;
          unsigned long long pv = __hip_atomic_load(pf2, __ATOMIC_RELAXED, __HIP_MEMORY_SCOPE_AGENT);
          for (uint32_t spins = 1;; ++spins) {
            bool found = false;
            if (lds_ld_u32(ptile_lds + 4u * slot2) == t2) {
              asm volatile("" ::: "memory");
              g = s_pfx[slot2];
              found = true;
            } else {
              g = rfl_u64(pv);
              if (granule_ok(p, g, 2)) {
                if (lane == 0) {
                  s_pfx[slot2] = g;
                  asm volatile("s_waitcnt lgkmcnt(0)" ::: "memory");
                  lds_st_u32(ptile_lds + 4u * slot2, t2);
                }
                found = true;
              } else if (GH_TILE_POLLDIV <= 1 || ((spins + (uint32_t)wid) % GH_TILE_POLLDIV) == 0u) {
                pv = __hip_atomic_load(pf2, __ATOMIC_RELAXED, __HIP_MEMORY_SCOPE_AGENT);
              }
            }
            if (found) break;
            if ((spins & 63u) == 0u) {
              if (__hip_atomic_load(p.status, __ATOMIC_RELAXED, __HIP_MEMORY_SCOPE_AGENT) & GH_ST_TIMEOUT) break;
              const unsigned long long t = wall_clock64();
              if (t0w == 0) {
                t0w = t;
              } else if (t - t0w > 400000000ull) {
                if (lane == 0) atomicOr(p.status, (unsigned)GH_ST_TIMEOUT);
                break;
              }
            }
            __builtin_amdgcn_s_sleep(1);
          }
          got = granule_ok(p, g, 2);
        }
      }
      asm volatile("" ::: "memory");
      goff = (g & GRAN_VMASK) + s_off[slot2 * NW + wid];
      if (GH_TILE_ABLATE & 32) goff &= ~15ull;
      n2 = s_tot[slot2 * NW + wid];
      if (wid == NW - 1 && t2 == p.ntiles - 1 && got && lane == 0) *p.total = goff + n2;
#if GH_TILE_STAMPS
      if (wid == 0 && lane == 0) p.tstamps[p.ntiles + t2] = __builtin_amdgcn_s_memrealtime() | ((unsigned long long)polled << 63);
#endif
      n2 = (!got || goff >= p.out_cap) ? 0u : (uint32_t)min<unsigned long long>(n2, p.out_cap - goff);
    }
    TSTAMP(4);
    if (!(GH_TILE_ABLATE & 8)) {
      tile_v4u cv[TILE_NS];
      uint32_t cb;
      copy_out_piece<TILE_NS, false>(p.out, region0 + buf * NW * p.stage_bytes, goff, n2, lane, cv, cb);
    }
    TSTAMP(5);
    const uint32_t st_t = GH_TILE_HOLD ? prevt : cur;
    const bool have_st = st_t < p.ntiles;
    const uint32_t st_tot = GH_TILE_HOLD ? wtp : wave_tot;
    const uint32_t st_slot = GH_TILE_HOLD ? slotp : slot;
    const bool staged = have_st && st_tot <= piece_cap;
    auto stage_or_store = [&](const uint32_t (&sow)[U][OW], const uint32_t (&scnt)[U], const uint32_t (&sbpos)[U],
                              int sgd) {
      if (have_st && !staged) {
        unsigned long long goffc = 0;
        bool got = true;
        if (lane == 0) {
          unsigned long long g = __hip_atomic_load(&p.prefix[st_t], __ATOMIC_RELAXED, __HIP_MEMORY_SCOPE_AGENT);
          if (!granule_ok(p, g, 2)) g = poll_granule(p, &p.prefix[st_t], 2);
          got = granule_ok(p, g, 2);
          asm volatile("" ::: "memory");
          goffc = (g & GRAN_VMASK) + s_off[st_slot * NW + wid];
          if (wid == NW - 1 && st_t == p.ntiles - 1 && got) *p.total = goffc + st_tot;
        }
        goffc = rfl_u64(goffc);
        if (__builtin_amdgcn_readfirstlane(got ? 1 : 0)) {
#pragma unroll
          for (int u = 0; u < U; ++u) store_direct(p.out, p.out_cap, goffc + sbpos[u], sow[u], scnt[u]);
        }
        __builtin_amdgcn_s_waitcnt(0x0F70);
      } else if (have_st && !(GH_TILE_ABLATE & 2)) {
        const uint32_t sbase = region0 + buf * NW * p.stage_bytes + STAGE_PAD;
        uint32_t o[U];
#pragma unroll
        for (int u = 0; u < U; ++u) o[u] = sbase + sbpos[u];
        stage_wave<U, OW>(sow, scnt, o, min(OW, (GRP * sgd + 3) >> 2));
      }
    };
    if constexpr (GH_TILE_HOLD) {
      stage_or_store(owp, cntp, bposp, gdp);
#pragma unroll
      for (int u = 0; u < U; ++u) {
        cntp[u] = cnt[u];
        bposp[u] = bpos[u];
#pragma unroll
        for (int k2 = 0; k2 < OW; ++k2) owp[u][k2] = ow[u][k2];
      }
      wtp = wave_tot;
      gdp = gdone;
    } else {
      stage_or_store(ow, cnt, bpos, gdone);
    }
    TSTAMP(6);
#if GH_TILE_STAMPS
    TSTAMP(7);
    TSTAMP(8);
    if (lane == 0 && (wid == 0 || wid == NW / 2) && k < 128) {
      uint4* st = p.stamps + (((unsigned long long)blockIdx.x * 2 + (wid ? 1 : 0)) * 128 + k) * 2;
      st[0] = make_uint4((uint32_t)(ts[1] - ts[0]), (uint32_t)(ts[2] - ts[1]), (uint32_t)(ts[3] - ts[2]),
                         (uint32_t)(ts[4] - ts[3]));
      st[1] = make_uint4((uint32_t)(ts[5] - ts[4]), (uint32_t)(ts[6] - ts[5]), (uint32_t)(ts[7] - ts[6]),
                         (uint32_t)(ts[8] - ts[7]));
    }
#endif
#pragma unroll
    for (int i = TILE_LAG - 1; i > 0; --i) th[i] = th[i - 1];
    th[0] = staged ? st_t : NONE;
    if constexpr (GH_TILE_HOLD) prevt = have_cur ? cur : NONE;
    cur = nxt < p.ntiles ? nxt : NONE;
    if constexpr (!GH_TILE_DYN) nxt += G;
    return true;
  };
  for (uint32_t k = 0;; k += NSET) {
    if (!body(std::integral_constant<int, 0>{}, k)) break;
    if constexpr (NSET == 2) {
      if (!body(std::integral_constant<int, NSET - 1>{}, k + 1)) break;
    }
  }
#if GH_TILE_STAMPS
  if (tid == 0) {
    wring[2] = __builtin_amdgcn_s_memtime();
    wring[3] = __builtin_amdgcn_s_memrealtime();
  }
#endif
}
```

Measured before the change: 2366.

## Strip dead tile-kernel variants and simplify segment loading to a single buffer set

Removes unused compile-time variants: dynamic ticket scheduling, hold/delay staging, the alternate LDS read paths, ds_write2, and extra prefetch. The per-tile load is reworked so each lane derives its segment start nibbles with a bitfield extract from a gap word and computes activity from the remaining segments in the tile, replacing the old per-segment gap lookup. The two alternating load buffer sets are collapsed into one loop body. This cuts code size and register pressure, but may lose some load/decode overlap. The load also relies on host padding for reads past the shard end.

```diff
diff --git a/cse375-finalproj-huffman-decoding_amd/csrc/gh_decode.hip b/cse375-finalproj-huffman-decoding_amd/csrc/gh_decode.hip
--- a/cse375-finalproj-huffman-decoding_amd/csrc/gh_decode.hip
+++ b/cse375-finalproj-huffman-decoding_amd/csrc/gh_decode.hip
@@ -864,7 +864,6 @@
     t.status = c->misc_at(1);
     t.total = (unsigned long long*)c->misc_at(2);
     t.stats = (unsigned long long*)c->misc_at(4);
-    t.tickets = (unsigned int*)(gran + 2ull * tp.ntiles);
     t.out_cap = sh.out_cap;
     t.nseg = sh.nseg;
     t.gap_nib0 = sh.gap_nib0;
diff --git a/cse375-finalproj-huffman-decoding_amd/csrc/gh_tile.hip b/cse375-finalproj-huffman-decoding_amd/csrc/gh_tile.hip
--- a/cse375-finalproj-huffman-decoding_amd/csrc/gh_tile.hip
+++ b/cse375-finalproj-huffman-decoding_amd/csrc/gh_tile.hip
@@ -24,40 +24,6 @@
 #define TSTAMP(i) (ts[i] = __builtin_amdgcn_s_memtime())
 #else
 #define TSTAMP(i) ((void)0)
-#endif
-#ifndef GH_TILE_CSUB
-#define GH_TILE_CSUB 0
-#endif
-#ifndef GH_TILE_CLDS
-#define GH_TILE_CLDS 0
-#endif
-#ifndef GH_TILE_LMAJ
-#define GH_TILE_LMAJ 1
-#endif
-#ifndef GH_TILE_POLLDIV
-#define GH_TILE_POLLDIV 1
-#endif
-#ifndef GH_TILE_DYN
-#define GH_TILE_DYN 0
-#endif
-constexpr int TILE_TAHEAD = 5;
-#ifndef GH_TILE_LATEP
-#define GH_TILE_LATEP 0
-#endif
-#ifndef GH_TILE_EPERM
-#define GH_TILE_EPERM 0
-#endif
-#ifndef GH_TILE_HOLD
-#define GH_TILE_HOLD 0
-#endif
-#ifndef GH_TILE_ALRD
-#define GH_TILE_ALRD 1
-#endif
-#ifndef GH_TILE_W2
-#define GH_TILE_W2 0
-#endif
-#ifndef GH_TILE_PF2
-#define GH_TILE_PF2 0
 #endif
 #ifndef GH_TILE_ABLATE
 #define GH_TILE_ABLATE 0
@@ -85,14 +51,13 @@
   unsigned int stage_bytes;
   unsigned int kbits_c;
   unsigned int fb_hi;
-  unsigned int* tickets;
   uint4* stamps;
   unsigned long long* tstamps;
 };
 
 inline size_t tile_lds_bytes(size_t lut_bytes, size_t stage_bytes) {
   return lut_bytes + TILE_LAG * (TILE_TB / 64) * stage_bytes + TILE_SLOTS * (2 * (TILE_TB / 64) + 1) * 4 +
-         TILE_SLOTS * 12 + 4 * (TILE_TB / 64) + 4 * TILE_SLOTS + 32;
+         TILE_SLOTS * 12 + 4 * (TILE_TB / 64) + 32;
 }
 
 __device__ __forceinline__ constexpr uint32_t perm_sel(int j) {
@@ -117,7 +82,6 @@
 template <int N>
 __device__ __forceinline__ void lds_wait_n(uint32_t& v) {
   static_assert(N >= 0 && N <= 3, "lgkmcnt 0..3");
-  if constexpr (GH_TILE_CLDS) return;
   if constexpr (N == 0) asm volatile("s_waitcnt lgkmcnt(0)" : "+v"(v)::"memory");
   else if constexpr (N == 1) asm volatile("s_waitcnt lgkmcnt(1)" : "+v"(v)::"memory");
   else if constexpr (N == 2) asm volatile("s_waitcnt lgkmcnt(2)" : "+v"(v)::"memory");
@@ -130,14 +94,9 @@
                                                    uint32_t laneoff, Mid&& mid) {
   constexpr int S = 4 * OW;
   constexpr int NG = (S + G - 1) / G;
-  constexpr int PLACE = GH_TILE_EPERM ? GH_TILE_EPERM : (G >= 4 ? 2 : 0);
+  constexpr bool PLACE = G >= 4;
   uint32_t q[U], ent[U];
-#if GH_TILE_CLDS
-  const __attribute__((address_space(3))) uint8_t* const lds0 = (const __attribute__((address_space(3))) uint8_t*)nullptr;
-  auto lut_rd = [&](uint32_t a) -> uint32_t { return *(const __attribute__((address_space(3))) uint32_t*)(lds0 + a); };
-#else
   auto lut_rd = [&](uint32_t a) -> uint32_t { return lds_u32_nowait(a); };
-#endif
 #pragma unroll
   for (int u = 0; u < U; ++u) {
     q[u] = q_init(act[u], start[u]);
@@ -174,20 +133,10 @@
           } else {
             lds_wait_n<U - 1>(ent[u]);
           }
-#if GH_TILE_CSUB
-          {
-            uint32_t nq;
-            const bool br = __builtin_sub_overflow(q[u], ent[u], &nq);
-            q[u] = nq;
-            cnt[u] = br ? (uint32_t)(pos + 1) : cnt[u];
-          }
-#else
           asm("v_sub_co_u32 %0, vcc, %0, %2\n\t"
               "v_cndmask_b32_e64 %1, %1, %3, vcc"
               : "+v"(q[u]), "+v"(cnt[u]) : "v"(ent[u]), "i"(pos + 1) : "vcc");
-#endif
           ow[u][pos >> 2] = __builtin_amdgcn_perm(ent[u], ow[u][pos >> 2], perm_sel(pos & 3));
-          if (PLACE == 1) asm volatile("" : "+v"(ow[u][pos >> 2]));
           if (!gend) {
             const uint32_t x = __builtin_amdgcn_alignbit(e[u][0], e[u][1], q[u]);
             ent[u] = lut_rd((x & amask) | laneoff);
@@ -204,7 +153,7 @@
         }
       }
     }
-    if (PLACE == 2) {
+    if (PLACE) {
 #pragma unroll
       for (int u = 0; u < U; ++u) {
         const int w0 = (gi * G) >> 2, w1 = min(OW - 1, (gi * G + G - 1) >> 2);
@@ -262,31 +211,11 @@
     sh[u] = 4u - ap;
   }
   auto dw = [&](int u, int m) { return __builtin_amdgcn_alignbyte(m < OW ? ow[u][m] : 0u, ow[u][m - 1], sh[u]); };
-  if constexpr (GH_TILE_W2) {
-#pragma unroll
-    for (int m = OW; m >= 1; m -= 2) {
-      if (m - 1 >= 1) {
-        if (m <= mmax) {
-#pragma unroll
-          for (int u = 0; u < U; ++u)
-            asm volatile("ds_write2_b32 %0, %1, %2 offset0:%3 offset1:%4" ::"v"(base[u]), "v"(dw(u, m)),
-                         "v"(dw(u, m - 1)), "i"(m), "i"(m - 1) : "memory");
-        } else if (m - 1 <= mmax) {
-#pragma unroll
-          for (int u = 0; u < U; ++u) lds_st32_m(base[u], dw(u, m - 1), m - 1);
-        }
-      } else if (m <= mmax) {
-#pragma unroll
-        for (int u = 0; u < U; ++u) lds_st32_m(base[u], dw(u, m), m);
-      }
-    }
-  } else {
-#pragma unroll
-    for (int m = OW; m >= 1; --m) {
-      if (m > mmax) continue;
-#pragma unroll
-      for (int u = 0; u < U; ++u) lds_st32_m(base[u], dw(u, m), m);
-    }
+#pragma unroll
+  for (int m = OW; m >= 1; --m) {
+    if (m > mmax) continue;
+#pragma unroll
+    for (int u = 0; u < U; ++u) lds_st32_m(base[u], dw(u, m), m);
   }
   uint32_t rd[U];
 #pragma unroll
@@ -328,112 +257,50 @@
     if (t < nh) k = lb + t;
     else if (t < nh + nt) k = 16u * ce + (t - nh);
   }
-  if constexpr (GH_TILE_ALRD) {
-    constexpr int CG = NS % 2 == 0 ? 2 : 1;
-    const uint32_t sh = (16u - lb) & 15u, r = sh & 3u, m = lb ? sh >> 2 : 4u;
-    if constexpr (GH_TILE_ALRD == 2) {
-      tile_v4u P[NS + 1];
-#pragma unroll
-      for (int i = 0; i <= NS; ++i) {
-        const uint32_t c = c0 + cf + (uint32_t)lane + 64u * (uint32_t)i;
-        const uint32_t a = stg + 16u * (c < ce + 1u ? c : cf);
-        asm volatile("ds_read_b128 %0, %1" : "=v"(P[i]) : "v"(a) : "memory");
-      }
+  constexpr int CG = NS % 2 == 0 ? 2 : 1;
+  const uint32_t sh = (16u - lb) & 15u, r = sh & 3u, m = lb ? sh >> 2 : 4u;
+#pragma unroll
+  for (int g0 = 0; g0 < NS; g0 += CG) {
+    tile_v4u pq[CG][2];
+#pragma unroll
+    for (int j = 0; j < CG; ++j) {
+      const int i = g0 + j;
+      const uint32_t c = c0 + cf + (uint32_t)lane + 64u * (uint32_t)i;
+      const uint32_t a = stg + 16u * (c < ce ? c : cf);
+      asm volatile("ds_read_b128 %0, %1" : "=v"(pq[j][0]) : "v"(a) : "memory");
+      asm volatile("ds_read_b128 %0, %1 offset:16" : "=v"(pq[j][1]) : "v"(a) : "memory");
+    }
+    if (g0 + CG >= NS) {
       if (PIN) asm volatile("ds_read_u8 %0, %1" : "+v"(b) : "v"(src + (k == OOB_OFF ? 0u : k)) : "memory");
       else asm volatile("ds_read_u8 %0, %1" : "=v"(b) : "v"(src + (k == OOB_OFF ? 0u : k)) : "memory");
-      asm volatile("s_waitcnt lgkmcnt(0)" ::: "memory");
-#pragma unroll
-      for (int i = 0; i <= NS; ++i) asm volatile("" : "+v"(P[i]));
-#pragma unroll
-      for (int i = 0; i < NS; ++i) {
-        tile_v4u Q;
-#pragma unroll
-        for (int d = 0; d < 4; ++d) {
-          const int nx = __builtin_amdgcn_update_dpp(0, (int)P[i + 1][d], 0x134, 0xf, 0xf, false);
-          Q[d] = (uint32_t)__builtin_amdgcn_update_dpp(nx, (int)P[i][d], 0x130, 0xf, 0xf, false);
+    }
+    asm volatile("s_waitcnt lgkmcnt(0)" ::: "memory");
+#pragma unroll
+    for (int j = 0; j < CG; ++j) asm volatile("" : "+v"(pq[j][0]), "+v"(pq[j][1]));
+    auto shift = [&](auto mc) {
+      constexpr int M = decltype(mc)::value;
+#pragma unroll
+      for (int j = 0; j < CG; ++j) {
+        if constexpr (M == 4) {
+          v[g0 + j] = pq[j][1];
+        } else {
+          auto W = [&](int q) -> uint32_t { return q < 4 ? pq[j][0][q] : pq[j][1][q - 4]; };
+#pragma unroll
+          for (int d = 0; d < 4; ++d) v[g0 + j][d] = __builtin_amdgcn_alignbyte(W(M + d + 1), W(M + d), r);
         }
-        auto W = [&](int q) -> uint32_t { return q < 4 ? P[i][q] : Q[q - 4]; };
-        switch (m) {
-          case 0:
-            for (int d = 0; d < 4; ++d) v[i][d] = __builtin_amdgcn_alignbyte(W(d + 1), W(d), r);
-            break;
-          case 1:
-            for (int d = 0; d < 4; ++d) v[i][d] = __builtin_amdgcn_alignbyte(W(d + 2), W(d + 1), r);
-            break;
-          case 2:
-            for (int d = 0; d < 4; ++d) v[i][d] = __builtin_amdgcn_alignbyte(W(d + 3), W(d + 2), r);
-            break;
-          case 3:
-            for (int d = 0; d < 4; ++d) v[i][d] = __builtin_amdgcn_alignbyte(W(d + 4), W(d + 3), r);
-            break;
-          default:
-            v[i] = Q;
-            break;
-        }
-        __builtin_amdgcn_raw_buffer_store_b128(v[i], rs, (int)off[i], 0, 2);
-      }
-      if (PIN) asm volatile("" : "+v"(b));
-      __builtin_amdgcn_raw_buffer_store_b8((uint8_t)b, rs, (int)k, 0, 2);
-      return;
-    }
-#pragma unroll
-    for (int g0 = 0; g0 < NS; g0 += CG) {
-      tile_v4u pq[CG][2];
-#pragma unroll
-      for (int j = 0; j < CG; ++j) {
-        const int i = g0 + j;
-        const uint32_t c = c0 + cf + (uint32_t)lane + 64u * (uint32_t)i;
-        const uint32_t a = stg + 16u * (c < ce ? c : cf);
-        asm volatile("ds_read_b128 %0, %1" : "=v"(pq[j][0]) : "v"(a) : "memory");
-        asm volatile("ds_read_b128 %0, %1 offset:16" : "=v"(pq[j][1]) : "v"(a) : "memory");
-      }
-      if (g0 + CG >= NS) {
-        if (PIN) asm volatile("ds_read_u8 %0, %1" : "+v"(b) : "v"(src + (k == OOB_OFF ? 0u : k)) : "memory");
-        else asm volatile("ds_read_u8 %0, %1" : "=v"(b) : "v"(src + (k == OOB_OFF ? 0u : k)) : "memory");
-      }
-      asm volatile("s_waitcnt lgkmcnt(0)" ::: "memory");
-#pragma unroll
-      for (int j = 0; j < CG; ++j) asm volatile("" : "+v"(pq[j][0]), "+v"(pq[j][1]));
-      auto shift = [&](auto mc) {
-        constexpr int M = decltype(mc)::value;
-#pragma unroll
-        for (int j = 0; j < CG; ++j) {
-          if constexpr (M == 4) {
-            v[g0 + j] = pq[j][1];
-          } else {
-            auto W = [&](int q) -> uint32_t { return q < 4 ? pq[j][0][q] : pq[j][1][q - 4]; };
-#pragma unroll
-            for (int d = 0; d < 4; ++d) v[g0 + j][d] = __builtin_amdgcn_alignbyte(W(M + d + 1), W(M + d), r);
-          }
-        }
-      };
-      switch (m) {
-        case 0: shift(std::integral_constant<int, 0>{}); break;
-        case 1: shift(std::integral_constant<int, 1>{}); break;
-        case 2: shift(std::integral_constant<int, 2>{}); break;
-        case 3: shift(std::integral_constant<int, 3>{}); break;
-        default: shift(std::integral_constant<int, 4>{}); break;
-      }
-#pragma unroll
-      for (int j = 0; j < CG; ++j) __builtin_amdgcn_raw_buffer_store_b128(v[g0 + j], rs, (int)off[g0 + j], 0, 2);
-    }
-    if (PIN) asm volatile("" : "+v"(b));
-    __builtin_amdgcn_raw_buffer_store_b8((uint8_t)b, rs, (int)k, 0, 2);
-    return;
-  }
-#pragma unroll
-  for (int i = 0; i < NS; ++i) {
-    const uint32_t c = c0 + cf + (uint32_t)lane + 64u * (uint32_t)i;
-    if (PIN) asm volatile("ds_read_b128 %0, %1" : "+v"(v[i]) : "v"(src + 16u * (c < ce ? c : cf)) : "memory");
-    else asm volatile("ds_read_b128 %0, %1" : "=v"(v[i]) : "v"(src + 16u * (c < ce ? c : cf)) : "memory");
-  }
-  if (PIN) asm volatile("ds_read_u8 %0, %1" : "+v"(b) : "v"(src + (k == OOB_OFF ? 0u : k)) : "memory");
-  else asm volatile("ds_read_u8 %0, %1" : "=v"(b) : "v"(src + (k == OOB_OFF ? 0u : k)) : "memory");
-  asm volatile("s_waitcnt lgkmcnt(0)" : "+v"(b)::"memory");
-#pragma unroll
-  for (int i = 0; i < NS; ++i) asm volatile("" : "+v"(v[i]));
-#pragma unroll
-  for (int i = 0; i < NS; ++i) __builtin_amdgcn_raw_buffer_store_b128(v[i], rs, (int)off[i], 0, 2);
+      }
+    };
+    switch (m) {
+      case 0: shift(std::integral_constant<int, 0>{}); break;
+      case 1: shift(std::integral_constant<int, 1>{}); break;
+      case 2: shift(std::integral_constant<int, 2>{}); break;
+      case 3: shift(std::integral_constant<int, 3>{}); break;
+      default: shift(std::integral_constant<int, 4>{}); break;
+    }
+#pragma unroll
+    for (int j = 0; j < CG; ++j) __builtin_amdgcn_raw_buffer_store_b128(v[g0 + j], rs, (int)off[g0 + j], 0, 2);
+  }
+  if (PIN) asm volatile("" : "+v"(b));
   __builtin_amdgcn_raw_buffer_store_b8((uint8_t)b, rs, (int)k, 0, 2);
 }
 
@@ -519,74 +386,11 @@
   }
 }
 
-template <int TB>
-__device__ __forceinline__ void tile_frontier_leader(const TileParams& p, uint32_t* s_w, int tid, int lane, int wid) {
-  constexpr int NW = TB / 64;
-  uint32_t F = 0;
-  unsigned long long R = 0, t0 = 0;
-  uint32_t* const s_first = s_w;
-  uint32_t* const s_sum = s_w + 2 * NW;
-  for (uint32_t pass = 0; F < p.ntiles; ++pass) {
-    const uint32_t t = F + (uint32_t)tid, pb = (pass & 1u) * NW;
-    bool in = false;
-    uint32_t v = 0;
-    if (t < p.ntiles) {
-      const unsigned long long g = __hip_atomic_load(&p.granules[t], __ATOMIC_RELAXED, __HIP_MEMORY_SCOPE_AGENT);
-      in = granule_ok(p, g, 1);
-      v = (uint32_t)(g & GRAN_VMASK);
-    }
-    const unsigned long long out = __ballot(!in);
-    if (lane == 0) s_first[pb + wid] = out ? (uint32_t)__builtin_ctzll(out) : 64u;
-    __syncthreads();
-    uint32_t m = (uint32_t)TB;
-#pragma unroll
-    for (int q = NW - 1; q >= 0; --q) {
-      const uint32_t f = s_first[pb + q];
-      m = f < 64u ? 64u * (uint32_t)q + f : m;
-    }
-    const uint32_t vv = (uint32_t)tid < m ? v : 0u;
-    const uint32_t incl = wave_incl_scan(vv);
-    if (lane == 63) s_sum[pb + wid] = incl;
-    __syncthreads();
-    unsigned long long before = 0, total = 0;
-#pragma unroll
-    for (int q = 0; q < NW; ++q) {
-      const uint32_t x = s_sum[pb + q];
-      before += (q < wid) ? x : 0u;
-      total += x;
-    }
-    if ((uint32_t)tid < m) {
-      __hip_atomic_store(&p.prefix[t], granule(p.epoch, 2, R + before + incl - vv), __ATOMIC_RELAXED,
-                         __HIP_MEMORY_SCOPE_AGENT);
-#if GH_TILE_STAMPS
-      p.tstamps[2 * p.ntiles + t] = __builtin_amdgcn_s_memrealtime();
-#endif
-    }
-    R += total;
-    F += m;
-    if (m == 0u) {
-      if (tid == 0) atomicAdd(p.stats + 1, 1ull);
-      if ((pass & 63u) == 0u) {
-        if (__hip_atomic_load(p.status, __ATOMIC_RELAXED, __HIP_MEMORY_SCOPE_AGENT) & GH_ST_TIMEOUT) return;
-        const unsigned long long tw = wall_clock64();
-        if (t0 == 0) {
-          t0 = tw;
-        } else if (tw - t0 > 400000000ull) {
-          if (tid == 0) atomicOr(p.status, (unsigned)GH_ST_TIMEOUT);
-          return;
-        }
-      }
-      __builtin_amdgcn_s_sleep(2);
-    } else {
-      t0 = 0;
-    }
-  }
-}
-
 template <int TB, int U, int GRP, int OW, int MINL>
 __global__ __launch_bounds__(TB) __attribute__((amdgpu_waves_per_eu(4, 4))) void gh_tile_kernel(const TileParams p) {
   static_assert(4 * OW >= (128 + MINL - 1) / MINL, "OW words hold every codeword a segment can start");
   static_assert(U <= TILE_U, "shapes of at most TILE_U segments per lane");
+  static_assert(TILE_U <= 4, "a lane reads up to U segments past the shard end: the host pads 16 zero words");
   constexpr int NW = TB / 64;
   extern __shared__ __attribute__((aligned(16))) uint8_t smem[];
   const uint32_t stage_lds = p.lut_bytes;
@@ -596,10 +400,8 @@
   unsigned long long* s_pfx = (unsigned long long*)(s_cnt + TILE_SLOTS);
   uint32_t* s_ptile = (uint32_t*)(s_pfx + TILE_SLOTS);
   uint32_t* s_lead = s_ptile + TILE_SLOTS;
-  uint32_t* s_ring = s_lead + NW;
   const uint32_t cnt_lds = (uint32_t)((uint8_t*)s_cnt - smem);
   const uint32_t ptile_lds = (uint32_t)((uint8_t*)s_ptile - smem);
-  const uint32_t ring_lds = (uint32_t)((uint8_t*)s_ring - smem);
 
   const int tid = threadIdx.x, lane = tid & 63, wid = tid >> 6;
 #if GH_TILE_STAMPS
@@ -611,12 +413,7 @@
 #endif
   const uint32_t D = gridDim.x - 1 - (p.idle_block < gridDim.x ? 1u : 0u);
   if (blockIdx.x == 0) {
-    if constexpr (GH_TILE_DYN) {
-      if (tid == 0) p.tickets[2u * ((p.epoch + 1u) & 1u)] = 0u;
-      tile_frontier_leader<TB>(p, (uint32_t*)smem, tid, lane, wid);
-    } else {
-      tile_round_leader<TB>(p, D, s_lead, tid, lane, wid);
-    }
+    tile_round_leader<TB>(p, D, s_lead, tid, lane, wid);
 #if GH_TILE_STAMPS
     if (tid == 0) {
       lring[2] = __builtin_amdgcn_s_memtime();
@@ -641,11 +438,6 @@
       s_cnt[tid] = 0;
       s_ptile[tid] = 0xFFFFFFFFu;
     }
-    if (GH_TILE_DYN && tid <= TILE_TAHEAD) {
-      const uint32_t b0 = blockIdx.x - 1 - (blockIdx.x > p.idle_block ? 1u : 0u);
-      const uint32_t tt = b0 + (uint32_t)tid * D;
-      s_ring[tid] = tt < p.ntiles ? tt : 0xFFFFFFFFu;
-    }
   }
   const uint32_t S = 30u - p.kbits - p.lgr;
   const uint32_t amask = (((1u << p.kbits) - 1u) << (2u + p.lgr)) & ((GH_TILE_ABLATE & 16) ? ~(1u << (2u + p.lgr)) : ~0u);
@@ -656,55 +448,42 @@
   const uint32_t nseg = (uint32_t)p.nseg;
   constexpr uint32_t NONE = 0xFFFFFFFFu;
   __syncthreads();
-  const uint32_t last_tile_k = GH_TILE_DYN ? p.ntiles + 2u * TILE_SLOTS
-                               : b < p.ntiles ? (p.ntiles - 1 - b) / G : NONE;
+  const uint32_t last_tile_k = b < p.ntiles ? (p.ntiles - 1 - b) / G : NONE;
   uint32_t cur = b, nxt = b + G;
-  const uint32_t dyn_base = (uint32_t)(TILE_TAHEAD + 1) * D;
-  uint32_t tk = 0;
-  bool tk_live = GH_TILE_DYN && dyn_base < p.ntiles;
-  unsigned int* const tctr = GH_TILE_DYN ? p.tickets + 2u * (p.epoch & 1u) : nullptr;
-  constexpr uint32_t CSTR = GH_TILE_LMAJ ? 1u : 64u;
-  const uint32_t lseg = (uint32_t)(wid * 64 * U) + (uint32_t)lane * (GH_TILE_LMAJ ? (uint32_t)U : 1u);
-  constexpr int NSET = GH_TILE_PF2 ? 2 : 1;
-  static_assert(!(GH_TILE_PF2 && (GH_TILE_DYN || GH_TILE_HOLD)), "PF2: static schedule, no hold");
-  uint4 wset[NSET][U];
-  uint32_t w4set[NSET][U], gwset[NSET][U];
-  auto load = [&](auto SS, uint32_t t) {
-    constexpr int SI = decltype(SS)::value;
-    uint4 (&w)[U] = wset[SI];
-    uint32_t (&w4)[U] = w4set[SI];
-    uint32_t (&gw)[U] = gwset[SI];
-    const uint32_t seg0 = min(t, p.ntiles - 1) * (uint32_t)(U * TB) + lseg;
-    if constexpr (GH_TILE_LMAJ) {
-      const uint32_t sb = min(seg0, nseg - 1);
-#pragma unroll
-      for (int u = 0; u < U; ++u) w[u] = *(const uint4*)(p.payload + 4ull * (sb + (uint32_t)u));
-      w4[U - 1] = p.payload[4ull * (sb + (uint32_t)U)];
-#pragma unroll
-      for (int u = 0; u < U; ++u) {
-        const uint32_t sc = sb + (uint32_t)u;
-        gw[u] = p.gaps[(p.gap_nib0 + (sc ? sc - 1u : 0u)) >> 3];
-      }
-    } else {
-#pragma unroll
-      for (int u = 0; u < U; ++u) {
-        const uint32_t sc = min(seg0 + (uint32_t)(64 * u), nseg - 1);
-        w[u] = *(const uint4*)(p.payload + 4ull * sc);
-        w4[u] = p.payload[4ull * sc + 4];
-        gw[u] = p.gaps[(p.gap_nib0 + (sc ? sc - 1u : 0u)) >> 3];
-      }
+  const uint32_t lseg = (uint32_t)(wid * 64 * U) + (uint32_t)lane * (uint32_t)U;
+  uint4 w[U];
+  uint32_t w4[U], gw[U];
+  static_assert((U * TB) % 8 == 0, "a tile's gap nibbles fill whole dwords");
+  uint32_t poff = 16u * lseg;
+  asm volatile("" : "+v"(poff));
+  uint32_t goffb[U];
+#pragma unroll
+  for (int u = 0; u < U; ++u) goffb[u] = ((p.gap_nib0 + lseg + (uint32_t)u + 7u) >> 3) * 4u;
+  const uint32_t gsh0 = 4u * ((p.gap_nib0 + lseg + 7u) & 7u);
+  const unsigned long long pay_bytes = 16ull * p.nseg + 64ull;
+  const uint32_t gap_bytes = 4u * (((p.gap_nib0 + nseg - 1u) >> 3) + 5u);
+  auto load = [&](uint32_t t, bool first) {
+    const uint32_t tt = (uint32_t)__builtin_amdgcn_readfirstlane((int)min(t, p.ntiles - 1));
+    const unsigned long long pb = (unsigned long long)tt * (unsigned long long)(16 * U * TB);
+    const unsigned long long prem = pay_bytes - pb;
+    const __amdgpu_buffer_rsrc_t rp = __builtin_amdgcn_make_buffer_rsrc(
+        (void*)((const uint8_t*)p.payload + pb), 0, (int)((uint32_t)(prem >> 32) ? 0xFFFFFFFFu : (uint32_t)prem), 0x00020000);
+    const uint32_t gb = tt ? tt * (uint32_t)(U * TB / 2) - 4u : 0u;
+    const __amdgpu_buffer_rsrc_t rg = __builtin_amdgcn_make_buffer_rsrc(
+        (void*)((const uint8_t*)p.gaps + gb), 0, (int)(gap_bytes - gb), 0x00020000);
+#pragma unroll
+    for (int u = 0; u < U; ++u) {
+      const tile_v4u x = __builtin_amdgcn_raw_buffer_load_b128(rp, (int)(poff + 16u * (uint32_t)u), 0, 0);
+      w[u] = make_uint4(x[0], x[1], x[2], x[3]);
+    }
+    w4[U - 1] = __builtin_amdgcn_raw_buffer_load_b32(rp, (int)(poff + 16u * (uint32_t)U), 0, 0);
+#pragma unroll
+    for (int u = 0; u < U; ++u) {
+      const uint32_t go = (first && tt == 0u) ? max(goffb[u], 4u) - 4u : goffb[u];
+      gw[u] = __builtin_amdgcn_raw_buffer_load_b32(rg, (int)go, 0, 0);
     }
   };
   const __amdgpu_buffer_rsrc_t rs_out = __builtin_amdgcn_make_buffer_rsrc(p.out, 0, 0x7FFFFFF0, 0x00020000);
-  auto ticket_op = [&]() {
-    if constexpr (GH_TILE_DYN) {
-      if (wid == 0 && tk_live) {
-        if (lane == 0) tk = atomicAdd(tctr, 1u);
-      } else {
-        __builtin_amdgcn_raw_buffer_store_b8((uint8_t)0, rs_out, (int)(OOB_OFF + 64u), 0, 2);
-      }
-    }
-  };
   auto junk_stores = [&]() {
     const __amdgpu_buffer_rsrc_t rs = rs_out;
 #pragma unroll
@@ -712,44 +491,24 @@
       __builtin_amdgcn_raw_buffer_store_b128(tile_v4u{0, 0, 0, 0}, rs, (int)(OOB_OFF + 16u * (uint32_t)i), 0, 2);
     __builtin_amdgcn_raw_buffer_store_b8((uint8_t)0, rs, (int)OOB_OFF, 0, 2);
   };
-  load(std::integral_constant<int, 0>{}, cur);
-  ticket_op();
+  load(cur, true);
   junk_stores();
-  if constexpr (GH_TILE_PF2) {
-    (void)__hip_atomic_load(&p.prefix[0], __ATOMIC_RELAXED, __HIP_MEMORY_SCOPE_AGENT);
-    (void)__hip_atomic_load(&p.prefix[0], __ATOMIC_RELAXED, __HIP_MEMORY_SCOPE_AGENT);
-    load(std::integral_constant<int, NSET - 1>{}, nxt);
-    junk_stores();
-  }
   if (cur >= p.ntiles) cur = NONE;
   uint32_t th[TILE_LAG];
 #pragma unroll
   for (int i = 0; i < TILE_LAG; ++i) th[i] = NONE;
-  uint32_t owp[U][OW], cntp[U], bposp[U], wtp = 0, prevt = NONE;
-  int gdp = 1;
-#pragma unroll
-  for (int u = 0; u < U; ++u) {
-    cntp[u] = 0;
-    bposp[u] = 0;
-#pragma unroll
-    for (int k2 = 0; k2 < OW; ++k2) asm volatile("" : "=v"(owp[u][k2]));
-  }
   uint32_t rank = 0;
   const uint32_t region0 = stage_lds + (uint32_t)wid * p.stage_bytes;
   const uint32_t piece_cap = p.stage_bytes - (uint32_t)(STAGE_PAD + 4 * OW + 4);
 #if GH_TILE_STAMPS
   unsigned long long ts[9];
 #endif
-  auto body = [&](auto SS, uint32_t k) -> bool {
-    constexpr int SI = decltype(SS)::value;
-    uint4 (&w)[U] = wset[SI];
-    uint32_t (&w4)[U] = w4set[SI];
-    uint32_t (&gw)[U] = gwset[SI];
+  auto body = [&](uint32_t k) -> bool {
     TSTAMP(0);
     const bool have_cur = cur < p.ntiles;
     const uint32_t t2 = th[TILE_LAG - 1];
     const bool have2 = t2 < p.ntiles;
-    bool pending = have_cur || (GH_TILE_HOLD && prevt < p.ntiles);
+    bool pending = have_cur;
 #pragma unroll
     for (int i = 0; i < TILE_LAG; ++i) pending |= th[i] < p.ntiles;
     if (!pending) return false;
@@ -757,32 +516,31 @@
       if (lane == 0) atomicOr(p.status, (unsigned)GH_ST_TIMEOUT);
       return false;
     }
-    const uint32_t slot = k % TILE_SLOTS, slot2 = (k + TILE_SLOTS - TILE_LAG - GH_TILE_HOLD) % TILE_SLOTS;
-    const uint32_t slotp = (k + TILE_SLOTS - 1) % TILE_SLOTS;
+    const uint32_t slot = k % TILE_SLOTS, slot2 = (k + TILE_SLOTS - TILE_LAG) % TILE_SLOTS;
     const uint32_t buf = k % TILE_LAG;
     if (rank >= 3) __builtin_amdgcn_s_setprio(3);
     else if (rank == 2) __builtin_amdgcn_s_setprio(2);
     else if (rank == 1) __builtin_amdgcn_s_setprio(1);
     else __builtin_amdgcn_s_setprio(0);
     unsigned long long* const pf2 = &p.prefix[have2 ? t2 : 0u];
-    unsigned long long gp0 = 0, gp = 0, gpl = 0;
+    unsigned long long gp0 = 0, gp = 0;
     if (!(GH_TILE_ABLATE & 4)) gp0 = __hip_atomic_load(pf2, __ATOMIC_RELAXED, __HIP_MEMORY_SCOPE_AGENT);
     auto mid = [&]() {
       if (!(GH_TILE_ABLATE & 4)) gp = __hip_atomic_load(pf2, __ATOMIC_RELAXED, __HIP_MEMORY_SCOPE_AGENT);
     };
-    const uint32_t seg0 = cur * (uint32_t)(U * TB) + lseg;
     uint32_t ow[U][OW], cnt[U];
     int gdone;
     {
       int start[U];
       bool act[U];
       uint32_t e[U][5];
+      const uint32_t rem = have_cur ? min(nseg - cur * (uint32_t)(U * TB), (uint32_t)(U * TB)) : 0u;
 #pragma unroll
       for (int u = 0; u < U; ++u) {
-        const uint32_t seg = seg0 + (uint32_t)u * CSTR;
-        act[u] = have_cur && seg < nseg;
-        start[u] = seg == 0 ? (int)p.first_start : (int)gap_nib(gw[u], p.gap_nib0 + seg - 1u);
-        make_ewin(w[u], (GH_TILE_LMAJ && u + 1 < U) ? w[u + 1 < U ? u + 1 : u].x : w4[u], start[u], S, e[u]);
+        act[u] = poff < 16u * (rem > (uint32_t)u ? rem - (uint32_t)u : 0u);
+        start[u] = (int)__builtin_amdgcn_ubfe(gw[u], gsh0 + 4u * (uint32_t)u, 4u);
+        if (u == 0) start[u] = (cur == 0u && poff == 0u) ? (int)p.first_start : start[u];
+        make_ewin(w[u], u + 1 < U ? w[u + 1 < U ? u + 1 : u].x : w4[u], start[u], S, e[u]);
       }
       TSTAMP(1);
       if (GH_TILE_ABLATE & 1) {
@@ -798,23 +556,10 @@
         gdone = decode_tile_rolling<GRP, U, OW, MINL>(e, start, act, ow, cnt, amask, laneoff, mid);
       }
     }
-    if constexpr (GH_TILE_DYN) {
-      if (wid == 0) {
-        uint32_t tpost = NONE;
-        if (lane == 0 && tk_live) tpost = dyn_base + tk < p.ntiles ? dyn_base + tk : NONE;
-        tpost = (uint32_t)__builtin_amdgcn_readfirstlane((int)tpost);
-        tk_live = tk_live && tpost != NONE;
-        if (lane == 0) lds_st_u32(ring_lds + 4u * ((k + 1u + TILE_TAHEAD) % TILE_SLOTS), tpost);
-      }
-      nxt = lds_ld_u32(ring_lds + 4u * ((k + 1u) % TILE_SLOTS));
-      nxt = (uint32_t)__builtin_amdgcn_readfirstlane((int)nxt);
-    }
-    if (GH_TILE_LATEP && !(GH_TILE_ABLATE & 4)) gpl = __hip_atomic_load(pf2, __ATOMIC_RELAXED, __HIP_MEMORY_SCOPE_AGENT);
-    load(SS, GH_TILE_PF2 ? nxt + G : nxt);
-    ticket_op();
+    load(nxt, false);
     TSTAMP(2);
     uint32_t bpos[U], wave_tot = 0;
-    if constexpr (GH_TILE_LMAJ) {
+    {
       uint32_t sl = 0;
 #pragma unroll
       for (int u = 0; u < U; ++u) sl += cnt[u];
@@ -826,15 +571,6 @@
         run += cnt[u];
       }
       wave_tot = (uint32_t)__builtin_amdgcn_readlane((int)incl, 63);
-    } else {
-#pragma unroll
-      for (int u = 0; u < U; ++u) bpos[u] = wave_incl_scan(cnt[u]);
-#pragma unroll
-      for (int u = 0; u < U; ++u) {
-        const uint32_t ct = (uint32_t)__builtin_amdgcn_readlane((int)bpos[u], 63);
-        bpos[u] += wave_tot - cnt[u];
-        wave_tot += ct;
-      }
     }
     uint32_t tile_total = 0;
     if (have_cur) {
@@ -873,7 +609,6 @@
       bool polled = false, got = true;
       (void)polled;
       if (!granule_ok(p, g, 2)) g = rfl_u64(gp);
-      if (GH_TILE_LATEP && !granule_ok(p, g, 2)) g = rfl_u64(gpl);
       {
         if (!granule_ok(p, g, 2)) {
           polled = true;
@@ -895,7 +630,7 @@
                   lds_st_u32(ptile_lds + 4u * slot2, t2);
                 }
                 found = true;
-              } else if (GH_TILE_POLLDIV <= 1 || ((spins + (uint32_t)wid) % GH_TILE_POLLDIV) == 0u) {
+              } else {
                 pv = __hip_atomic_load(pf2, __ATOMIC_RELAXED, __HIP_MEMORY_SCOPE_AGENT);
               }
             }
@@ -932,13 +667,12 @@
       copy_out_piece<TILE_NS, false>(p.out, region0 + buf * NW * p.stage_bytes, goff, n2, lane, cv, cb);
     }
     TSTAMP(5);
-    const uint32_t st_t = GH_TILE_HOLD ? prevt : cur;
+    const uint32_t st_t = cur;
     const bool have_st = st_t < p.ntiles;
-    const uint32_t st_tot = GH_TILE_HOLD ? wtp : wave_tot;
-    const uint32_t st_slot = GH_TILE_HOLD ? slotp : slot;
+    const uint32_t st_tot = wave_tot;
+    const uint32_t st_slot = slot;
     const bool staged = have_st && st_tot <= piece_cap;
-    auto stage_or_store = [&](const uint32_t (&sow)[U][OW], const uint32_t (&scnt)[U], const uint32_t (&sbpos)[U],
-                              int sgd) {
+    {
       if (have_st && !staged) {
         unsigned long long goffc = 0;
         bool got = true;
@@ -953,30 +687,16 @@
         goffc = rfl_u64(goffc);
         if (__builtin_amdgcn_readfirstlane(got ? 1 : 0)) {
 #pragma unroll
-          for (int u = 0; u < U; ++u) store_direct(p.out, p.out_cap, goffc + sbpos[u], sow[u], scnt[u]);
+          for (int u = 0; u < U; ++u) store_direct(p.out, p.out_cap, goffc + bpos[u], ow[u], cnt[u]);
         }
         __builtin_amdgcn_s_waitcnt(0x0F70);
       } else if (have_st && !(GH_TILE_ABLATE & 2)) {
         const uint32_t sbase = region0 + buf * NW * p.stage_bytes + STAGE_PAD;
         uint32_t o[U];
 #pragma unroll
-        for (int u = 0; u < U; ++u) o[u] = sbase + sbpos[u];
-        stage_wave<U, OW>(sow, scnt, o, min(OW, (GRP * sgd + 3) >> 2));
-      }
-    };
-    if constexpr (GH_TILE_HOLD) {
-      stage_or_store(owp, cntp, bposp, gdp);
-#pragma unroll
-      for (int u = 0; u < U; ++u) {
-        cntp[u] = cnt[u];
-        bposp[u] = bpos[u];
-#pragma unroll
-        for (int k2 = 0; k2 < OW; ++k2) owp[u][k2] = ow[u][k2];
-      }
-      wtp = wave_tot;
-      gdp = gdone;
-    } else {
-      stage_or_store(ow, cnt, bpos, gdone);
+        for (int u = 0; u < U; ++u) o[u] = sbase + bpos[u];
+        stage_wave<U, OW>(ow, cnt, o, min(OW, (GRP * gdone + 3) >> 2));
+      }
     }
     TSTAMP(6);
 #if GH_TILE_STAMPS
@@ -993,16 +713,12 @@
 #pragma unroll
     for (int i = TILE_LAG - 1; i > 0; --i) th[i] = th[i - 1];
     th[0] = staged ? st_t : NONE;
-    if constexpr (GH_TILE_HOLD) prevt = have_cur ? cur : NONE;
     cur = nxt < p.ntiles ? nxt : NONE;
-    if constexpr (!GH_TILE_DYN) nxt += G;
+    nxt += G;
     return true;
   };
-  for (uint32_t k = 0;; k += NSET) {
-    if (!body(std::integral_constant<int, 0>{}, k)) break;
-    if constexpr (NSET == 2) {
-      if (!body(std::integral_constant<int, NSET - 1>{}, k + 1)) break;
-    }
+  for (uint32_t k = 0;; ++k) {
+    if (!body(k)) break;
   }
 #if GH_TILE_STAMPS
   if (tid == 0) {
```

Result: no change. 2379 (median of 6 runs) (+0.5%).
